# XinMing0411/AC-VAE

Hardware: AMD Instinct MI355X
Metric: train-step captions/s (and audio-sec/s) at B=32, 1/2/4/8 MI355X (higher is better)
Workload: dtype f32

## Files before the change

### acvae_amd/_lib.py

```python
import ctypes
import os
import re
import threading

import numpy as np
import torch

from . import streams

_HERE = os.path.dirname(os.path.abspath(__file__))
HEADER = os.path.join(os.path.dirname(_HERE), "include", "acvae_hip.h")
LIB_PATH = os.path.join(_HERE, "libacvae_hip.so")

_CT = {"int": ctypes.c_int, "int64_t": ctypes.c_int64, "float": ctypes.c_float, "double": ctypes.c_double,
       "uint64_t": ctypes.c_uint64}
ERRORS = {-1: "ACVAE_EINVAL (bad dims / null pointer)", -2: "ACVAE_EALIGN (alignment)",
          -3: "ACVAE_EUNSUPPORTED", -4: "ACVAE_EWORKSPACE (workspace too small)"}


def parse_header(path=HEADER):
    src = open(path).read()
    src = re.sub(r"/\*.*?\*/", "", src, flags=re.S)
    protos = {}
    for m in re.finditer(r"\b(int|int64_t)\s+(acvae_\w+)\s*\(([^)]*)\)\s*;", src):
# ... 5 lines not shown
                if "*" in a:
                    alist.append((a.split("*")[-1].strip(), ctypes.c_void_p))
                else:
                    toks = a.replace("const ", "").split()
                    alist.append((toks[-1], _CT[toks[0]]))
        protos[name] = (_CT[ret], alist)
    enums = {}
    for m in re.finditer(r"enum\s+\w*\s*\{([^}]*)\}", src):
        val = -1
        for item in m.group(1).split(","):
            item = item.strip()
            if not item:
                continue
            if "=" in item:
                k, v = item.split("=")
                val = int(v.strip(), 0)
                enums[k.strip()] = val
            else:
                val += 1
                enums[item] = val
    return protos, enums


PROTOS, ENUMS = parse_header()
_defs = dict(re.findall(r"#define\s+(ACVAE_\w+)\s+(\d+)", open(HEADER).read()))
ENUMS_TEXT_N = int(_defs["ACVAE_TEXT_NPARAMS"])
ENC_NPARAMS = int(_defs["ACVAE_ENC_NPARAMS"])
ENC_BF16 = int(_defs["ACVAE_ENC_BF16"])
FLAG_NO_PERSIST = int(_defs["ACVAE_FLAG_NO_PERSIST"])
FLAG_DEFER_PARAM_GRADS = int(_defs["ACVAE_FLAG_DEFER_PARAM_GRADS"])
FLAG_NO_ATTN_SPLIT = int(_defs["ACVAE_FLAG_NO_ATTN_SPLIT"])
FLAG_TEST_STALL = int(_defs["ACVAE_FLAG_TEST_STALL"])
FLAG_ROLLOUT_GRAD = int(_defs["ACVAE_FLAG_ROLLOUT_GRAD"])
_lib = None


class options:
    persist = os.environ.get("ACVAE_DECODE_PERSIST", "1") != "0"
    defer = os.environ.get("ACVAE_DECODE_DEFER", "1") != "0"
    attn_split = True
    test_stall = False


class override:
    _lock = threading.Lock()
    _open = []
    _base = None

    def __init__(self, **kw):
        self.kw = kw

    @staticmethod
    def _apply():
        vals = dict(override._base)
        for o in override._open:
            vals.update(o.kw)
        for k, v in vals.items():
            setattr(options, k, v)

    def __enter__(self):
        with override._lock:
            if not override._open:
                override._base = {k: v for k, v in vars(options).items() if not k.startswith("_")}
            override._open.append(self)
            override._apply()
        return self

    def __exit__(self, *exc):
        with override._lock:
            override._open.remove(self)
            override._apply()
        return False


def call_flags(defer=False):
    f = 0
    if not options.persist:
        f |= FLAG_NO_PERSIST
    if not options.attn_split:
        f |= FLAG_NO_ATTN_SPLIT
    if options.test_stall:
        f |= FLAG_TEST_STALL
    if defer and options.defer:
        f |= FLAG_DEFER_PARAM_GRADS
    return f


def use_library(path):
    global LIB_PATH
    if _lib is not None:
        raise RuntimeError("acvae_amd._lib.use_library() must come before the first library call")
    LIB_PATH = os.path.abspath(path)


def lib():
    global _lib
    if _lib is None:
        if not os.path.exists(LIB_PATH):
            raise RuntimeError(f"{LIB_PATH} not built: run `python -c 'import __graft_entry__ as g; g.build()'` "
                               "(the AC-VAE HIP path has no CPU fallback)")
        _lib = ctypes.CDLL(LIB_PATH)
        for name, (ret, args) in PROTOS.items():
            fn = getattr(_lib, name)
            fn.restype = ret
            fn.argtypes = [t for _, t in args]
    return _lib


def ptr_table(tensors):
    return (ctypes.c_void_p * len(tensors))(*[None if t is None else t.data_ptr() for t in tensors])


def _conv(x):
    if isinstance(x, torch.Tensor):
        return x.data_ptr()
# ... 199 lines not shown
```

### acvae_amd/csrc/conv.h

```cpp
#pragma once
#include <hip/hip_runtime.h>
#include <stdint.h>
#include "common.h"
#include "job_table.h"
#include "bn_bwd.h"

struct DropoutSpec {
  float p;
  const uint8_t* mask;
  uint64_t seed;
  uint32_t site;
};

enum { UP_PLAIN = 0, UP_POOL = 1, UP_DROP = 2 };

namespace acvae {
int conv3x3_igemm(const float* X, const float* scale, const float* shift, const float* Wp, float* Y, float* partials,
                  int N, int H, int W, int Cin, int Cout, hipStream_t st);
int conv_partials_rows(int N, int H, int W);
int conv3x3_igemm_bf16(const bf16_t* X, const float* scale, const float* shift, const bf16_t* Wp, bf16_t* Y,
                       float* partials, int N, int H, int W, int Cin, int Cout, hipStream_t st);
long conv3x3_wgrad_bf16_slab_floats(int N, int H, int W, int Cin, int Cout);
int conv3x3_wgrad_bf16_splits(int N, int H, int W, int Cin, int Cout);
int conv3x3_wgrad_bf16_launch(const bf16_t* dY, const bf16_t* X, const float* scale, const float* shift, float* slab, int N,
// ... 51 lines not shown
bool colsum_batch_plan(ColsumBatch& b, long dpart_doubles, long* dsum_doubles);
int conv1_first_blocks(int N, int T);
template <class TY>
int conv1_first_fwd(const float* x, const float* scale0, const float* shift0, const float* W1, TY* Y,
                    float* partials, int N, int T, int F, hipStream_t st);
template <class TY>
int conv1_first_bwd(const float* x, const float* scale0, const float* shift0, const float* mean0, const float* invstd0,
                    const float* W1, const TY* dY, float* dw_part, float* bn_part, float* dW1, float* dgamma0,
                    float* dbeta0, double* dpart, int N, int T, int F, hipStream_t st, const BnBwdApply* bn = nullptr);
template <class T>
int bn_relu_pool(const T* Y, const float* scale, const float* shift, T* P, int N, int H, int W, int C,
                 DropoutSpec drop, hipStream_t st, bool pool = true);
int bn_bwd_blocks(int N, int H, int W, int C);
template <class T>
int bn_bwd(const T* Y, const T* dO, int upstream, const float* scale, const float* shift, const float* mean,
           const float* invstd, float* partials, float* sum_g, float* sum_gy, T* dY, double* dpart, int N, int H,
           int W, int C, DropoutSpec drop, hipStream_t st, bool batch_stats = true, int ready_rows = 0);
template <class T>
int bn_bwd_sums(const T* Y, const T* dO, int upstream, const float* scale, const float* shift, const float* mean,
                const float* invstd, float* partials, float* sum_g, float* sum_gy, double* dpart, int N, int H, int W, int C,
                DropoutSpec drop, hipStream_t st, int ready_rows = 0);
template <class T>
int relu_mask(const T* Y, const float* scale, const float* shift, uint8_t* out, int N, int H, int W, int C, hipStream_t st);
template <class T>
int freq_mean(const T* P, float* out, long rows, int Fp, int C, hipStream_t st);
template <class T>
int freq_mean_bwd(const float* dae, T* dP, long rows, int Fp, int C, hipStream_t st);
int time_pool(const float* ae, float* out, int N, int S, int C, DropoutSpec drop, hipStream_t st);
int relu_dropout(float* x, int total, DropoutSpec drop, hipStream_t st);
}

int acvae_gemm_nt_dual(const float* A1, int64_t lda1, const float* B1, int64_t ldb1, int K1, const float* A2,
                       int64_t lda2, const float* B2, int64_t ldb2, int K2, const float* bias, float* C, int64_t ldc,
                       int M, int N, int accumulate, hipStream_t st, float* skws = nullptr);
int acvae_gemm_nt_pair(const float* A0, int64_t lda0, const float* B0, int64_t ldb0, int K0, const float* bias0, float* C0,
                       int64_t ldc0, int N0, int acc0, const float* A1, int64_t lda1, const float* B1, int64_t ldb1, int K1,
                       const float* bias1, float* C1, int64_t ldc1, int N1, int acc1, int M, hipStream_t st);
constexpr int TN_TICKETS = 256;
int acvae_gemm_tn_fused(const float* A, int64_t lda, const float* B, int64_t ldb, float* C, int64_t ldc, int M, int N, int K,
                        int accumulate, float* ws, int64_t ws_bytes, hipStream_t st);
struct TnJob {
  const float* A; long lda; const float* B; long ldb; float* C; long ldc;
  int M, N, K, k_per, slices, gx, gy, tk0;
  long slab0;
};
using TnGroup = acvae::RangeTable<TnJob, 8, int>;
bool acvae_gemm_tn_group_add(TnGroup& g, const float* A, long lda, const float* B, long ldb, float* C, long ldc, int M, int N,
                             int K);
long acvae_gemm_tn_group_plan(TnGroup& g);
int acvae_gemm_tn_group(TnGroup& g, float* ws, int64_t ws_bytes, hipStream_t st);
long acvae_skinny_ws_floats();
long acvae_skinny_ticket_words();
int acvae_skinny_ws_reset(float* ws, hipStream_t st);
struct TransposeJob { const float* in; long ld_in; float* out; long ld_out; int rows, cols; };
using TransposeBatch = acvae::RangeTable<TransposeJob, 12, int>;
int acvae_transpose_batch(TransposeBatch& b, hipStream_t st);
```

### acvae_amd/csrc/decoder.hip

```cpp
#include <cstdlib>
#include <vector>
#include "common.h"
#include "constrain.h"
#include "conv.h"
#include "rnn.h"
#include "decode_persist.h"
#include "text_common.h"

namespace {

inline int gemm2(const float* A1, long lda1, const float* B1, long ldb1, int K1, const float* A2, long lda2,
                 const float* B2, long ldb2, int K2, const float* bias, float* C, long ldc, int M, int N, int acc,
                 const Ctx& st) {
  if (M <= 64)
    return acvae_gemm_nt_dual(A1, lda1, B1, ldb1, K1, A2, lda2, B2, ldb2, K2, bias, C, ldc, M, N, acc, st.s, st.skws);
  ACVAE_TRY(acvae_gemm_nt_dual(A1, lda1, B1, ldb1, K1, nullptr, 0, nullptr, 0, 0, bias, C, ldc, M, N, acc, st.s, st.skws));
  return acvae_gemm_nt_dual(A2, lda2, B2, ldb2, K2, nullptr, 0, nullptr, 0, 0, nullptr, C, ldc, M, N, 1, st.s, st.skws);
}
struct TnWs { float* p; long bytes; };
inline int gemm_tn(const float* A, long lda, const float* B, long ldb, float* C, long ldc, int M, int N, int K, TnWs ws,
                   hipStream_t st) {
  return acvae_gemm_tn_fused(A, lda, B, ldb, C, ldc, M, N, K, 0, ws.p, ws.bytes, st);
}
struct TnBatch {
// ... 526 lines not shown
  if (truncate && (sample_method == ACVAE_SAMPLE_GREEDY || (flags & ACVAE_FLAG_ROLLOUT_GRAD))) return ACVAE_EINVAL;
  if (emb_keep && !(emb_drop_p > 0.f && emb_drop_p <= 1.f)) return ACVAE_EINVAL;
  if (sample_method != ACVAE_SAMPLE_GREEDY &&
      ((sample_method != ACVAE_SAMPLE_GUMBEL && sample_method != ACVAE_SAMPLE_MULTINOMIAL) || !sample_noise ||
       !(temp > 0.f)))
    return ACVAE_EINVAL;
  DecLayout L;
  ACVAE_TRY(dec_layout(N, Tc, S, E, H, A, V, Eenc, L));
  if (!params || !mem_in || !mem_lens || !eps_p || !logits || !outputs || !seqs || !sampled_logprobs || !attn_w ||
      !p_means || !p_logs || !p_z || !saved_v || !scratch_v)
    return ACVAE_EINVAL;
  const bool train = caps != nullptr;
  const bool rollout_grad = !train && (flags & ACVAE_FLAG_ROLLOUT_GRAD);
  if (train && (!lens1 || !q_z || !ss_flags_host || !dis_flags_host || !p_means_utt)) return ACVAE_EINVAL;
  if (train && H != E) return ACVAE_EUNSUPPORTED;
  if (saved_bytes < L.saved_total * 4 || scratch_bytes < dec_scratch_floats(L) * 4) return ACVAE_EWORKSPACE;
  float* sv = (float*)saved_v;
  float* sc = (float*)scratch_v;
  auto P = [&](int i) { return (const float*)params[i]; };
  const int R = N * Tc, Hp = E;
  const bool has_ln = Eenc != E || params[TP_LN_W] != nullptr;
  bool teacher = train, prior_feeds_decoder = !train;
  if (train)
    for (int t = 0; t < Tc; ++t) {
      teacher = teacher && ss_flags_host[t] != 0;
      prior_feeds_decoder = prior_feeds_decoder || dis_flags_host[t] != 0;
    }
  Ctx st{(hipStream_t)stream, sc + L.skws};
  const Fork fork{st.s, (aux_stream && teacher) ? (hipStream_t)aux_stream : st.s};
  Ctx sp{fork.aux, sc + L.skws_p};
  acvae::PdPlan pd_plan{};
  const bool persist_fwd = teacher && !prior_feeds_decoder && !(flags & ACVAE_FLAG_NO_PERSIST) && H == E &&
                           acvae::decode_fwd_resident(N, Tc, S, E, H, A, pd_plan);
  const bool attws_ready = !persist_fwd && L.attfws_bytes > 0;
  {
    acvae::ZeroBatch zb;
    zb_skinny(zb, st.skws); zb_skinny(zb, sp.skws);
    if (attws_ready) { zb.add(sc + L.attfws_d, 256); zb.add(sc + L.attfws_p, 256); }
    if (persist_fwd) { zb.add(sc + L.pd_cnt, pd_plan.counter_words); flags |= ACVAE_FLAG_INT_CNT_ZEROED; }
    zb.add(sc + L.h0, (long)N * (H > Hp ? H : Hp));
    ACVAE_TRY(acvae::zero_batch(zb, st.s));
  }

  int64_t* words = (int64_t*)(sv + L.words);
  const float* mem = has_ln ? sv + L.mem : mem_in;
  float* encproj_d = sv + L.encproj_d;
  float* encproj_p = sv + L.encproj_p;
  float* qd = sv + L.qd;
  float* qp = sv + L.qp;
  float* attw_p = sv + L.attw_p;
  float* rnn_d = sv + L.rnn_d;
  float* rnn_p = sv + L.rnn_p;
  float* gi_d = sc + L.gi_d;
  float* gh_d = sc + L.gh_d;
  float* gates_p = sc + L.gates_p;
  float* ml = sc + L.ml;
  float* zeros = sc + L.h0;
  uint8_t* unfinished = (uint8_t*)(sv + L.unfinished);
  const long ld3E = (long)Tc * 3 * E;

  if (has_ln) ACVAE_TRY(gemm(mem_in, Eenc, P(TP_LN_W), Eenc, P(TP_LN_B), sv + L.mem, E, N * S, E, Eenc, 0, st));
  auto encproj_prior = [&](const Ctx& c) -> int {
    return gemm(mem, E, P(TP_P_ATT_W) + E, 2 * E, P(TP_P_ATT_B), encproj_p, E, N * S, E, E, 0, c);
  };
  auto encproj_dec = [&]() -> int {
    return gemm(mem, E, P(TP_DEC_ATT_W) + H, E + H, P(TP_DEC_ATT_B), encproj_d, A, N * S, A, E, 0, st);
  };

  auto rows_of = [&](int cnt) { return cnt == Tc ? R : N; };
  auto ldof = [&](int cnt, long C) { return cnt == Tc ? C : (long)Tc * C; };
  auto prior_pre = [&](int t0, int cnt) -> int {
    const int M = rows_of(cnt);
    ACVAE_TRY(acvae::embed_gather(words + t0, cnt == Tc ? 1 : Tc, P(TP_P_EMB), V, rnn_p + (long)t0 * 3 * E,
                                  ldof(cnt, 3 * E), M, E, sp));
    ACVAE_TRY(gemm(rnn_p + (long)t0 * 3 * E, ldof(cnt, 3 * E), P(TP_P_ATT_W), 2 * E, nullptr, qp + (long)t0 * E,
                   ldof(cnt, E), M, E, E, 0, sp));
    ACVAE_TRY(acvae_attn_fwd(qp + (long)t0 * E, (long)Tc * E, E, encproj_p, mem, mem_lens, P(TP_P_ATT_V),
                             rnn_p + (long)t0 * 3 * E + E, ld3E, 3 * E, attw_p + (long)t0 * S, (long)Tc * S, S, N, cnt, S,
                             E, E, (cnt == 1 && attws_ready) ? sc + L.attfws_p : nullptr, L.attfws_bytes, sp, flags));
    ACVAE_TRY(gemm(rnn_p + (long)t0 * 3 * E, ldof(cnt, 3 * E), P(TP_P_WIH), 3 * E, P(TP_P_BIH),
                   gates_p + (long)t0 * 4 * Hp, ldof(cnt, 4 * Hp), M, 4 * Hp, 2 * E, 0, sp));
    return ACVAE_OK;
  };
  float* hp_all = sv + L.hp_all;
  float* c_all = sv + L.c_all;
  float* hpprev = sv + L.hpprev;
  float* lstm_save = sv + L.lstm_save;
  auto prior_step = [&](int t) -> int {
    const float* hprev = t ? hp_all + (long)(t - 1) * Hp : zeros;
    const long ldh = t ? (long)Tc * Hp : Hp;
    const float* cprev = t ? c_all + (long)(t - 1) * Hp : nullptr;
    if (t == 0) ACVAE_TRY(acvae::copy_rows(rnn_p + 2 * E, ld3E, nullptr, 0, N, E, sp));
    ACVAE_TRY(gemm2(rnn_p + (long)t * 3 * E + 2 * E, ld3E, P(TP_P_WIH) + 2 * E, 3 * E, E, hprev, ldh, P(TP_P_WHH), Hp,
                    Hp, P(TP_P_BHH), gates_p + (long)t * 4 * Hp, (long)Tc * 4 * Hp, N, 4 * Hp, 1, sp));
    ACVAE_TRY(acvae::lstm_fwd(gates_p + (long)t * 4 * Hp, (long)Tc * 4 * Hp, cprev, (long)Tc * Hp,
                              hp_all + (long)t * Hp, (long)Tc * Hp, c_all + (long)t * Hp, (long)Tc * Hp,
                              lstm_save + (long)t * 5 * Hp, (long)Tc * 5 * Hp, N, Hp, sp));
    ACVAE_TRY(gemm(hp_all + (long)t * Hp, (long)Tc * Hp, P(TP_P_ML_W), Hp, P(TP_P_ML_B), ml, 2 * E, N, 2 * E, Hp, 0, sp));
    float* z2 = (t + 1 < Tc) ? rnn_p + (long)(t + 1) * 3 * E + 2 * E : nullptr;
    ACVAE_TRY(acvae_reparam_fwd(ml, 2 * E, eps_p + (long)t * N * E, E, p_means + (long)t * E, p_logs + (long)t * E,
                                p_z + (long)t * E, (long)Tc * E, z2, ld3E, N, E, sp));
    return ACVAE_OK;
  };
  auto dec_pre = [&](int t0, int cnt) -> int {
    const int M = rows_of(cnt);
    ACVAE_TRY(acvae::embed_gather(words + t0, cnt == Tc ? 1 : Tc, P(TP_DEC_EMB), V, rnn_d + (long)t0 * 3 * E,
                                  ldof(cnt, 3 * E), M, E, st));
    if (emb_keep)
      ACVAE_TRY(acvae::dropout_rows(rnn_d + (long)t0 * 3 * E, ld3E, 3 * E, emb_keep + (long)t0 * N * E, E, (long)N * E,
                                    emb_drop_p < 1.f ? 1.f / (1.f - emb_drop_p) : 0.f, N, cnt, E, st));
    if (cnt == Tc && train && !prior_feeds_decoder) {
      ACVAE_TRY(acvae::copy_rows(rnn_d + 2 * E, 3 * E, q_z, E, R, E, st));
    } else {
      for (int t = t0; t < t0 + cnt; ++t) {
        const float* zsrc = (train && !dis_flags_host[t]) ? q_z : p_z;
        ACVAE_TRY(acvae::copy_rows(rnn_d + (long)t * 3 * E + 2 * E, ld3E, zsrc + (long)t * E, (long)Tc * E, N, E, st));
      }
    }
    ACVAE_TRY(gemm2(rnn_d + (long)t0 * 3 * E, ldof(cnt, 3 * E), P(TP_DEC_WIH), 3 * E, E,
                    rnn_d + (long)t0 * 3 * E + 2 * E, ldof(cnt, 3 * E), P(TP_DEC_WIH) + 2 * E, 3 * E, E, P(TP_DEC_BIH),
                    gi_d + (long)t0 * 3 * H, ldof(cnt, 3 * H), M, 3 * H, 0, st));
    return ACVAE_OK;
  };
  float* gru_save = sv + L.gru_save;
  float* hprev_d = sv + L.hprev_d;
  const bool pair_ok = N <= 64;
  auto dec_step = [&](int t) -> int {
    const float* hprev = t ? outputs + (long)(t - 1) * H : zeros;
    const long ldh = t ? (long)Tc * H : H;
    if (pair_ok) {
      ACVAE_TRY(acvae_gemm_nt_pair(hprev, ldh, P(TP_DEC_ATT_W), E + H, H, nullptr, qd + (long)t * A, (long)Tc * A, A, 0,
                                   hprev, ldh, P(TP_DEC_WHH), H, H, P(TP_DEC_BHH), gh_d, 3 * H, 3 * H, 0, N, st));
    } else {
      ACVAE_TRY(gemm(hprev, ldh, P(TP_DEC_ATT_W), E + H, nullptr, qd + (long)t * A, (long)Tc * A, N, A, H, 0, st));
      ACVAE_TRY(gemm(hprev, ldh, P(TP_DEC_WHH), H, P(TP_DEC_BHH), gh_d, 3 * H, N, 3 * H, H, 0, st));
    }
    ACVAE_TRY(acvae_attn_fwd(qd + (long)t * A, (long)Tc * A, A, encproj_d, mem, mem_lens, P(TP_DEC_ATT_V),
// ... 11 lines not shown
    TransposeBatch tb;
    tb.add({P(TP_DEC_CLS_W), H, sv + L.wt_cls, V, V, H});
    tb.add({P(TP_DEC_WIH), 3 * E, sv + L.wt_dih, 3 * H, 3 * H, 3 * E});
    tb.add({P(TP_DEC_WHH), H, sv + L.wt_dhh, 3 * H, 3 * H, H});
    tb.add({P(TP_DEC_ATT_W), E + H, sv + L.wt_datt, A, A, E + H});
    tb.add({P(TP_P_WIH), 3 * E, sv + L.wt_pih, 4 * Hp, 4 * Hp, 3 * E});
    tb.add({P(TP_P_WHH), Hp, sv + L.wt_phh, 4 * Hp, 4 * Hp, Hp});
    tb.add({P(TP_P_ML_W), Hp, sv + L.wt_pml, 2 * E, 2 * E, Hp});
    tb.add({P(TP_P_ATT_W), 2 * E, sv + L.wt_patt, E, E, 2 * E});
    if (train) tb.add({P(TP_MLO_W), H, sv + L.wt_mlo, 2 * E, 2 * E, H});
    return acvae_transpose_batch(tb, ts);
  };
  float* lse = sv + L.lse;
  auto classify = [&](int t0, int cnt) -> int {
    const int M = rows_of(cnt);
    ACVAE_TRY(gemm(outputs + (long)t0 * H, ldof(cnt, H), P(TP_DEC_CLS_W), H, P(TP_DEC_CLS_B), logits + (long)t0 * V,
                   ldof(cnt, V), M, V, H, 0, st));
    if (con.on())
      ACVAE_TRY(acvae::constrain_rows(logits + (long)t0 * V, (long)Tc * V, seqs, Tc, t0, N, V, end_idx, con, st.s));
    ACVAE_TRY(acvae_row_logsoftmax_argmax(logits + (long)t0 * V, (long)Tc * V, V, seqs + t0, sampled_logprobs + t0,
                                          lse + t0, Tc, 1, N, cnt, V, st));
    if (truncate)
      ACVAE_TRY(acvae_sample_next_word_truncated(logits + (long)t0 * V, (long)Tc * V, V, sample_noise + (long)t0 * N * V,
                                                 V, (long)N * V, sample_method, temp, seqs + t0, sampled_logprobs + t0,
                                                 Tc, 1, N, cnt, V, top_k, top_p, kept ? kept + t0 : nullptr, st));
    else if (sample_method != ACVAE_SAMPLE_GREEDY)
      ACVAE_TRY(acvae_sample_next_word(logits + (long)t0 * V, (long)Tc * V, V, sample_noise + (long)t0 * N * V, V,
                                       (long)N * V, sample_method, temp, seqs + t0, sampled_logprobs + t0, Tc, 1, N, cnt,
                                       V, st));
    return ACVAE_OK;
  };

  if (teacher) {
    ACVAE_TRY(acvae::gather_words(caps, ld_caps, 1, words, N, Tc, st));
    ACVAE_TRY(fork.begin());
    ACVAE_TRY(encproj_prior(sp));
    ACVAE_TRY(encproj_dec());
    ACVAE_TRY(prior_pre(0, Tc));
    if (prior_feeds_decoder) {
      for (int t = 0; t < Tc; ++t) ACVAE_TRY(prior_step(t));
      ACVAE_TRY(fork.join());
      ACVAE_TRY(dec_pre(0, Tc));
      for (int t = 0; t < Tc; ++t) ACVAE_TRY(dec_step(t));
    } else if (persist_fwd) {
      ACVAE_TRY(dec_pre(0, Tc));
      ACVAE_TRY(acvae::copy_rows(rnn_p + 2 * E, ld3E, nullptr, 0, N, E, sp));
      ACVAE_TRY(fork.join());
      PdParams pd{};
      pd.w_att = P(TP_DEC_ATT_W); pd.w_hh = P(TP_DEC_WHH); pd.b_hh = P(TP_DEC_BHH); pd.w_ih = P(TP_DEC_WIH);
      pd.att_v = P(TP_DEC_ATT_V);
      pd.pw_ih = P(TP_P_WIH); pd.pw_hh = P(TP_P_WHH); pd.pb_hh = P(TP_P_BHH); pd.w_ml = P(TP_P_ML_W); pd.b_ml = P(TP_P_ML_B);
      pd.encproj = encproj_d; pd.mem = mem; pd.mem_lens = mem_lens; pd.gi = gi_d; pd.gates_p = gates_p;
      pd.eps_p = eps_p; pd.zeros = zeros;
      pd.qd = qd; pd.gh = gh_d; pd.rnn_d = rnn_d; pd.attn_w = attn_w; pd.outputs = outputs; pd.gru_save = sv + L.gru_save;
      pd.hprev_d = sv + L.hprev_d; pd.rnn_p = rnn_p; pd.hp_all = sv + L.hp_all; pd.c_all = sv + L.c_all;
      pd.lstm_save = sv + L.lstm_save; pd.p_means = p_means; pd.p_logs = p_logs; pd.p_z = p_z;
      pd.cnt = (unsigned*)(sc + L.pd_cnt);
      ACVAE_TRY(acvae::decode_persist_fwd(pd, pd_plan, st.s, flags));
    } else {
      ACVAE_TRY(dec_pre(0, Tc));
      for (int t = 0; t < Tc; ++t) {
        ACVAE_TRY(prior_step(t));
        ACVAE_TRY(dec_step(t));
      }
    }
    ACVAE_TRY(transposes(sp.s));
    ACVAE_TRY(classify(0, Tc));
// ... 57 lines not shown
                                          void* stream, void* aux_stream, int sample_method, float temp,
                                          const float* sample_noise, const uint8_t* emb_keep, float emb_drop_p, int flags,
                                          int top_k, float top_p, int32_t* kept) {
  return decode_fwd_driver(params, mem_in, mem_lens, caps, ld_caps, lens1, q_z, eps_p, ss_flags_host, dis_flags_host, logits,
                           outputs, seqs, sampled_logprobs, attn_w, p_means, p_logs, p_z, p_means_utt, h_final, hp_final,
                           cp_final, saved_v, saved_bytes, scratch_v, scratch_bytes, N, Tc, S, E, H, A, V, Eenc, start_idx,
                           end_idx, stream, aux_stream, sample_method, temp, sample_noise, emb_keep, emb_drop_p, flags,
                           top_k, top_p, kept, acvae::Constraints{});
}

extern "C" int acvae_decode_fwd_constrained(const void* const* params, const float* mem_in, const int64_t* mem_lens,
                                            const int64_t* caps, int64_t ld_caps, const int64_t* lens1, const float* q_z,
                                            const float* eps_p, const int* ss_flags_host, const int* dis_flags_host,
                                            float* logits, float* outputs, int64_t* seqs, float* sampled_logprobs,
                                            float* attn_w, float* p_means, float* p_logs, float* p_z, float* p_means_utt,
                                            float* h_final, float* hp_final, float* cp_final, void* saved_v,
                                            int64_t saved_bytes, void* scratch_v, int64_t scratch_bytes, int N, int Tc,
                                            int S, int E, int H, int A, int V, int Eenc, int start_idx, int end_idx,
                                            void* stream, void* aux_stream, int sample_method, float temp,
                                            const float* sample_noise, const uint8_t* emb_keep, float emb_drop_p, int flags,
                                            int top_k, float top_p, int32_t* kept, float repetition_penalty,
                                            int no_repeat_ngram_size, int min_length, const int* suppress_host,
                                            int n_suppress) {
  acvae::Constraints con;
  con.repetition_penalty = repetition_penalty; con.no_repeat_ngram_size = no_repeat_ngram_size;
  con.min_length = min_length; con.suppress = suppress_host; con.n_suppress = n_suppress;
  return decode_fwd_driver(params, mem_in, mem_lens, caps, ld_caps, lens1, q_z, eps_p, ss_flags_host, dis_flags_host, logits,
                           outputs, seqs, sampled_logprobs, attn_w, p_means, p_logs, p_z, p_means_utt, h_final, hp_final,
                           cp_final, saved_v, saved_bytes, scratch_v, scratch_bytes, N, Tc, S, E, H, A, V, Eenc, start_idx,
                           end_idx, stream, aux_stream, sample_method, temp, sample_noise, emb_keep, emb_drop_p, flags,
                           top_k, top_p, kept, con);
}

extern "C" int acvae_decode_bwd_defers(const int* dis_flags_host, int Tc, void* stream, void* aux_stream, int flags) {
  if (!(flags & ACVAE_FLAG_DEFER_PARAM_GRADS) || !aux_stream || aux_stream == stream || !dis_flags_host) return 0;
  for (int t = 0; t < Tc; ++t)
    if (dis_flags_host[t] != 0) return 0;
  return 1;
}

extern "C" int acvae_decode_bwd(const void* const* params, void* const* grads, const float* mem_in,
                                const int64_t* mem_lens, const int64_t* lens1, const float* eps_p,
                                const int* dis_flags_host, const float* outputs, const float* attn_w,
                                const float* p_logs, const float* d_logits, const float* d_outputs_ext,
                                const float* d_p_means, const float* d_p_logs, const float* d_p_z,
                                const float* d_p_means_utt, float* d_mem_in, float* d_q_z, void* saved_v,
                                int64_t saved_bytes, void* scratch_v, int64_t scratch_bytes, int N, int Tc, int S, int E,
                                int H, int A, int V, int Eenc, void* stream, void* aux_stream, const uint8_t* emb_keep,
                                float emb_drop_p, int flags) {
  if (emb_keep && !(emb_drop_p > 0.f && emb_drop_p <= 1.f)) return ACVAE_EINVAL;
  DecLayout L;
  ACVAE_TRY(dec_layout(N, Tc, S, E, H, A, V, Eenc, L));
  const bool rollout = (flags & ACVAE_FLAG_ROLLOUT_GRAD) != 0;
  if (!params || !grads || !mem_in || !mem_lens || !eps_p || !outputs || !attn_w || !p_logs || !d_mem_in || !saved_v ||
      !scratch_v)
    return ACVAE_EINVAL;
  if (rollout ? d_p_means_utt != nullptr : (!lens1 || !dis_flags_host || !d_q_z)) return ACVAE_EINVAL;
  if (saved_bytes < L.saved_total * 4 || scratch_bytes < dec_scratch_floats(L) * 4) return ACVAE_EWORKSPACE;
  float* sv = (float*)saved_v;
  float* sc = (float*)scratch_v;
  std::vector<int> rollout_flags;
  if (rollout) {
    rollout_flags.assign(Tc, 1);
    dis_flags_host = rollout_flags.data();
  }
  bool prior_feeds_decoder = false;
  for (int t = 0; t < Tc; ++t) prior_feeds_decoder = prior_feeds_decoder || dis_flags_host[t] != 0;
  Ctx st{(hipStream_t)stream, sc + L.skws};
  const Fork fork{st.s, aux_stream ? (hipStream_t)aux_stream : st.s};
  Ctx sp{fork.aux, sc + L.skws_p};
  auto P = [&](int i) { return (const float*)params[i]; };
  auto G = [&](int i) { return (float*)grads[i]; };
  const int R = N * Tc, Hp = E;
  const bool defer = acvae_decode_bwd_defers(dis_flags_host, Tc, stream, aux_stream, flags) != 0;
  const bool has_ln = Eenc != E || params[TP_LN_W] != nullptr;
  TnWs tn{sc + L.tn, L.tn_floats * 4};
  TnWs tn_p{sc + L.tn_p, L.tn_p_floats * 4};
  double* dpart = (double*)(sc + L.dpart);
  double* dpart_p = (double*)(sc + L.dpart_p);
  const acvae::PbPlan pb_plan = acvae::decode_bwd_plan(N, Tc, S, E, H, A);
  const bool persist_bwd = !prior_feeds_decoder && !(flags & ACVAE_FLAG_NO_PERSIST) && acvae::decode_bwd_resident(pb_plan);
  {
    acvae::ZeroBatch zb;
    zb_skinny(zb, st.skws); zb_skinny(zb, sp.skws); zb_colsum(zb, dpart); zb_colsum(zb, dpart_p); zb_tn(zb, tn); zb_tn(zb, tn_p);
    if (persist_bwd) {
      zb.add(sc + L.pd_cnt_b, pb_plan.counter_words);
      zb.add(sc + L.dmem_p, (long)N * S * E);
      if (pb_plan.rc_splits > 1) zb.add(sc + L.dqd, (long)R * A);
      flags |= ACVAE_FLAG_INT_CNT_ZEROED;
    }
    zb.add(G(TP_DEC_EMB), (long)V * E); zb.add(G(TP_P_EMB), (long)V * E);
    ACVAE_TRY(acvae::zero_batch(zb, st.s));
  }
  const int64_t* words = (const int64_t*)(sv + L.words);
  const float* mem = has_ln ? sv + L.mem : mem_in;
  float* rnn_d = sv + L.rnn_d;
  float* rnn_p = sv + L.rnn_p;

  float *wt_cls = sv + L.wt_cls, *wt_dih = sv + L.wt_dih, *wt_dhh = sv + L.wt_dhh, *wt_datt = sv + L.wt_datt;
  float *wt_pih = sv + L.wt_pih, *wt_phh = sv + L.wt_phh, *wt_pml = sv + L.wt_pml, *wt_patt = sv + L.wt_patt;
  float *wt_mlo = sv + L.wt_mlo, *wt_ln = sc + L.wt_ln;
  int64_t* words_c = (int64_t*)(sc + L.words_c);
  ACVAE_TRY(acvae::gather_words(words, Tc, 1, words_c, N, Tc, st));
  ACVAE_TRY(fork.begin());

  float* d_out = sc + L.d_out;
  if (d_outputs_ext) ACVAE_TRY(acvae::copy_rows(d_out, H, d_outputs_ext, H, R, H, st));
  else ACVAE_TRY(zero(d_out, (long)R * H, st));
// ... 37 lines not shown
  float* dh = sc + L.dh_a;
  float* dh2 = sc + L.dh_b;
  const float* gru_save = sv + L.gru_save;
  const float* hprev_d = sv + L.hprev_d;
  const float* qd = sv + L.qd;
  auto dec_begin = [&]() -> int {
    ACVAE_TRY(zero(dencproj, (long)N * S * A, st));
    ACVAE_TRY(zero(dvpart, (long)N * A, st));
    ACVAE_TRY(zero(dmem, (long)N * S * E, st));
    ACVAE_TRY(zero(dh, (long)N * H, st));
    return ACVAE_OK;
  };
  float* drnn = sc + L.drnn;
  float* dz_dec = sc + L.dz_dec;
  int dv_rows = N;
  auto dec_bptt = [&](int t) -> int {
    ACVAE_TRY(acvae::gru_bwd(dh, H, d_out + (long)t * H, (long)Tc * H, gru_save + (long)t * 4 * H, (long)Tc * 4 * H,
                             hprev_d + (long)t * H, (long)Tc * H, dgi + (long)t * 3 * H, (long)Tc * 3 * H,
                             dgh + (long)t * 3 * H, (long)Tc * 3 * H, dh2, H, nullptr, t, N, H, st));
    ACVAE_TRY(gemm(dgi + (long)t * 3 * H, (long)Tc * 3 * H, wt_dih + (long)E * 3 * H, 3 * H, nullptr, dctx, E, N, E,
                   3 * H, 0, st));
    ACVAE_TRY(acvae_attn_bwd(dctx, E, 0, qd + (long)t * A, (long)Tc * A, A, sv + L.encproj_d, mem, mem_lens,
                             P(TP_DEC_ATT_V), attn_w + (long)t * S, (long)Tc * S, S, dqd + (long)t * A, (long)Tc * A, A,
                             dencproj, dmem, dvpart, sc + L.attws, L.attws_bytes, N, 1, S, A, E, st));
    ACVAE_TRY(gemm2(dgh + (long)t * 3 * H, (long)Tc * 3 * H, wt_dhh, 3 * H, 3 * H, dqd + (long)t * A, (long)Tc * A,
                    wt_datt, A, A, nullptr, dh2, H, N, H, 1, st));
    float* tmp = dh; dh = dh2; dh2 = tmp;
    return ACVAE_OK;
  };
  auto dec_memgrad = [&]() -> int {
    return gemm(dencproj, A, wt_datt + (long)H * A, A, nullptr, dmem, E, N * S, E, A, 1, st);
  };
  auto dec_dz = [&](const Ctx& c) -> int {
    ACVAE_TRY(gemm(dgi, 3 * H, wt_dih + (long)2 * E * 3 * H, 3 * H, nullptr, dz_dec, E, R, E, 3 * H, 0, c));
    if (!d_q_z) return ACVAE_OK;
    if (!prior_feeds_decoder) {
      ACVAE_TRY(acvae::copy_rows(d_q_z, E, dz_dec, E, R, E, c));
    } else {
      for (int t = 0; t < Tc; ++t)
        ACVAE_TRY(acvae::copy_rows(d_q_z + (long)t * E, (long)Tc * E, dis_flags_host[t] ? nullptr : dz_dec + (long)t * E,
                                   (long)Tc * E, N, E, c));
    }
    return ACVAE_OK;
  };
  auto dec_tn = [&](TnBatch& tb) -> int {
    ACVAE_TRY(tb.add(dgi, 3 * H, rnn_d, 3 * E, G(TP_DEC_WIH), 3 * E, 3 * H, 3 * E, R));
    ACVAE_TRY(tb.add(dgh, 3 * H, hprev_d, H, G(TP_DEC_WHH), H, 3 * H, H, R));
    ACVAE_TRY(tb.add(dqd, A, hprev_d, H, G(TP_DEC_ATT_W), E + H, A, H, R));
    return tb.add(dencproj, A, mem, E, G(TP_DEC_ATT_W) + H, E + H, A, E, N * S);
  };
  auto dec_params = [&](const Ctx& c, TnWs ws, double* dp, bool with_dz = true, bool with_tn = true) -> int {
    if (with_tn) {
      TnBatch tb{{}, ws, c};
      ACVAE_TRY(dec_tn(tb));
      ACVAE_TRY(tb.launch());
    }
    {
      acvae::ColsumBatch cb;
      cb.add({dgi, R, 3 * H, G(TP_DEC_BIH)}); cb.add({dgh, R, 3 * H, G(TP_DEC_BHH)});
      cb.add({dencproj, N * S, A, G(TP_DEC_ATT_B)}); cb.add({dvpart, dv_rows, A, G(TP_DEC_ATT_V)});
      ACVAE_TRY(acvae::colsum_batch(cb, dp, L.dpart_doubles, c));
    }
    ACVAE_TRY(gemm(dgi, 3 * H, wt_dih, 3 * H, nullptr, drnn, E, R, E, 3 * H, 0, c));
    if (emb_keep)
      ACVAE_TRY(acvae::dropout_rows(drnn, (long)Tc * E, E, emb_keep, E, (long)N * E, emb_drop_p < 1.f ? 1.f / (1.f - emb_drop_p) : 0.f, N, Tc, E, c));
    if (with_dz) ACVAE_TRY(dec_dz(c));
// ... 21 lines not shown
  auto prior_begin = [&]() -> int {
  for (int t = 0; t < Tc; ++t) {
    ACVAE_TRY(acvae::copy_rows(dpz + (long)t * E, (long)Tc * E, d_p_z ? d_p_z + (long)t * E : nullptr, (long)Tc * E, N, E,
                               sp));
    if (dis_flags_host[t])
      ACVAE_TRY(acvae::add_rows(dpz + (long)t * E, (long)Tc * E, dz_dec + (long)t * E, (long)Tc * E, N, E, sp));
  }
  ACVAE_TRY(zero(dmem_p, (long)N * S * E, sp));
  ACVAE_TRY(zero(dhp, (long)N * Hp, sp));
  ACVAE_TRY(zero(dc, (long)N * Hp, sp));
  ACVAE_TRY(zero(dlz, (long)N * E, sp));
    return ACVAE_OK;
  };
  auto prior_bptt = [&](int t) -> int {
    ACVAE_TRY(acvae::add_rows(dlz, E, dpz + (long)t * E, (long)Tc * E, N, E, sp));
    ACVAE_TRY(acvae_reparam_bwd(dlz, E, d_p_means ? d_p_means + (long)t * E : nullptr,
                                d_p_logs ? d_p_logs + (long)t * E : nullptr, (long)Tc * E, p_logs + (long)t * E,
                                (long)Tc * E, eps_p + (long)t * N * E, E, dml_all + (long)t * 2 * E, (long)Tc * 2 * E, N,
                                E, sp));
    ACVAE_TRY(gemm(dml_all + (long)t * 2 * E, (long)Tc * 2 * E, wt_pml, 2 * E, nullptr, dhp, Hp, N, Hp, 2 * E, 1, sp));
    ACVAE_TRY(acvae::lstm_bwd(dhp, Hp, dc, Hp, lstm_save + (long)t * 5 * Hp, (long)Tc * 5 * Hp,
                              t ? c_all + (long)(t - 1) * Hp : nullptr, (long)Tc * Hp, dgates + (long)t * 4 * Hp,
                              (long)Tc * 4 * Hp, dc2, Hp, N, Hp, sp));
    ACVAE_TRY(gemm(dgates + (long)t * 4 * Hp, (long)Tc * 4 * Hp, wt_phh, 4 * Hp, nullptr, dhp2, Hp, N, Hp, 4 * Hp, 0, sp));
    ACVAE_TRY(gemm(dgates + (long)t * 4 * Hp, (long)Tc * 4 * Hp, wt_pih + (long)2 * E * 4 * Hp, 4 * Hp, nullptr, dlz2, E,
                   N, E, 4 * Hp, 0, sp));
    float* tmp = dhp; dhp = dhp2; dhp2 = tmp;
    tmp = dc; dc = dc2; dc2 = tmp;
    tmp = dlz; dlz = dlz2; dlz2 = tmp;
    return ACVAE_OK;
  };
  float* dqp = sc + L.dqp;
  auto prior_memgrad = [&]() -> int {
    ACVAE_TRY(gemm(dgates, 4 * Hp, wt_pih, 4 * Hp, nullptr, drnn_p, 3 * E, R, 2 * E, 4 * Hp, 0, sp));
    ACVAE_TRY(zero(dencproj_p, (long)N * S * E, sp));
    ACVAE_TRY(zero(dvpart_p, (long)N * E, sp));
    ACVAE_TRY(acvae_attn_bwd(drnn_p + E, (long)Tc * 3 * E, 3 * E, sv + L.qp, (long)Tc * E, E, sv + L.encproj_p, mem,
                             mem_lens, P(TP_P_ATT_V), sv + L.attw_p, (long)Tc * S, S, dqp, (long)Tc * E, E, dencproj_p,
                             dmem_p, dvpart_p, sc + L.attws_p, L.attws_bytes, N, Tc, S, E, E, sp));
    return gemm(dencproj_p, E, wt_patt + (long)E * E, E, nullptr, dmem_p, E, N * S, E, E, 1, sp);
  };
  auto prior_tn_bptt = [&](TnBatch& tb) -> int {
    ACVAE_TRY(tb.add(dgates, 4 * Hp, rnn_p, 3 * E, G(TP_P_WIH), 3 * E, 4 * Hp, 3 * E, R));
    ACVAE_TRY(tb.add(dgates, 4 * Hp, hpprev, Hp, G(TP_P_WHH), Hp, 4 * Hp, Hp, R));
    return tb.add(dml_all, 2 * E, hp_all, Hp, G(TP_P_ML_W), Hp, 2 * E, Hp, R);
  };
  auto prior_params = [&](bool with_bptt_tn = true) -> int {
    {
      TnBatch tb{{}, tn_p, sp};
      if (with_bptt_tn) ACVAE_TRY(prior_tn_bptt(tb));
      ACVAE_TRY(tb.add(dqp, E, rnn_p, 3 * E, G(TP_P_ATT_W), 2 * E, E, E, R));
      ACVAE_TRY(tb.add(dencproj_p, E, mem, E, G(TP_P_ATT_W) + E, 2 * E, E, E, N * S));
      ACVAE_TRY(tb.launch());
    }
    {
      acvae::ColsumBatch cb;
      cb.add({dml_all, R, 2 * E, G(TP_P_ML_B)}); cb.add({dgates, R, 4 * Hp, G(TP_P_BIH), G(TP_P_BHH)});
      cb.add({dencproj_p, N * S, E, G(TP_P_ATT_B)}); cb.add({dvpart_p, N, E, G(TP_P_ATT_V)});
      ACVAE_TRY(acvae::colsum_batch(cb, dpart_p, L.dpart_doubles, sp));
    }
    ACVAE_TRY(gemm(dqp, E, wt_patt, E, nullptr, drnn_p, 3 * E, R, E, E, 1, sp));
    return acvae::embed_scatter(words_c, drnn_p, 3 * E, G(TP_P_EMB), V, R, E, sp);
  };
  bool early_tn = false;
  if (prior_feeds_decoder) {
    ACVAE_TRY(dec_begin());
    for (int t = Tc - 1; t >= 0; --t) ACVAE_TRY(dec_bptt(t));
    ACVAE_TRY(dec_memgrad());
    ACVAE_TRY(dec_params(st, tn, dpart));
    if (fork.on()) ACVAE_TRY(Fork::edge(st.s, sp.s));
    ACVAE_TRY(prior_begin());
    for (int t = Tc - 1; t >= 0; --t) ACVAE_TRY(prior_bptt(t));
    ACVAE_TRY(prior_memgrad());
    ACVAE_TRY(prior_params());
  } else if (persist_bwd) {
    PbParams pb{};
    pb.wt_dhh = wt_dhh; pb.wt_datt = wt_datt; pb.wt_dih = wt_dih; pb.wt_phh = wt_phh; pb.wt_pih = wt_pih; pb.wt_pml = wt_pml;
    pb.att_v = P(TP_DEC_ATT_V);
    pb.encproj = sv + L.encproj_d; pb.mem = mem; pb.qd = qd; pb.attn_w = attn_w; pb.gru_save = gru_save; pb.hprev_d = hprev_d;
    pb.lstm_save = lstm_save; pb.c_all = c_all; pb.p_logs = p_logs; pb.eps_p = eps_p; pb.mem_lens = mem_lens;
    pb.d_out = d_out; pb.d_p_z = d_p_z; pb.d_p_means = d_p_means; pb.d_p_logs = d_p_logs;
    pb.dgi = dgi; pb.dgh = dgh; pb.dqd = dqd; pb.dctx = drnn;
    pb.dencproj = dencproj; pb.dmem = dmem; pb.dvpart = dvpart; pb.dgates = dgates; pb.dml_all = dml_all; pb.dhp = dhp;
    float* part = sc + L.pd_part;
    pb.dctx_part = part + pb_plan.dctx_part_off; pb.dhp_part = part + pb_plan.dhp_part_off; pb.dml_part = part + pb_plan.dml_part_off;
    pb.cnt = (unsigned*)(sc + L.pd_cnt_b);
    pb.dqd_part = sc + L.pd_dqd; pb.ctx = rnn_d + E;
    ACVAE_TRY(acvae::decode_persist_bwd(pb, pb_plan, st.s, flags));
    dv_rows = pb_plan.dv_rows;
    ACVAE_TRY(dec_memgrad());
    if (fork.on()) ACVAE_TRY(Fork::edge(st.s, sp.s));
    ACVAE_TRY(prior_memgrad());
    if (!defer) {
      ACVAE_TRY(dec_params(st, tn, dpart));
      ACVAE_TRY(prior_params());
    } else {
      TnBatch tb{{}, tn, st.s};
      ACVAE_TRY(dec_tn(tb));
      ACVAE_TRY(prior_tn_bptt(tb));
      ACVAE_TRY(tb.launch());
      early_tn = true;
    }
  } else {
    ACVAE_TRY(dec_begin());
    ACVAE_TRY(prior_begin());
    for (int t = Tc - 1; t >= 0; --t) {
      ACVAE_TRY(dec_bptt(t));
      ACVAE_TRY(prior_bptt(t));
    }
    ACVAE_TRY(dec_memgrad());
    ACVAE_TRY(prior_memgrad());
    if (!defer) {
      ACVAE_TRY(dec_params(st, tn, dpart));
      ACVAE_TRY(prior_params());
    }
  }
  ACVAE_TRY(fork.join());
  ACVAE_TRY(acvae::add_rows(dmem, E, dmem_p, E, N * S, E, st));
  if (has_ln) {
    ACVAE_TRY(transp(P(TP_LN_W), Eenc, wt_ln, E, E, Eenc, st));
    ACVAE_TRY(gemm(dmem, E, wt_ln, E, nullptr, d_mem_in, Eenc, N * S, Eenc, E, 0, st));
    ACVAE_TRY(gemm_tn(dmem, E, mem_in, Eenc, G(TP_LN_W), Eenc, E, Eenc, N * S, tn, st));
    ACVAE_TRY(acvae::colsum2(dmem, N * S, E, dpart, G(TP_LN_B), nullptr, 0, st));
  } else {
    ACVAE_TRY(acvae::copy_rows(d_mem_in, E, dmem, E, N * S, E, st));
  }
  if (defer) {
    ACVAE_TRY(dec_dz(st));
    ACVAE_TRY(Fork::edge(st.s, sp.s));
    ACVAE_TRY(dec_params(sp, tn_p, dpart_p, false, !early_tn));
    ACVAE_TRY(prior_params(!early_tn));
  }
  return ACVAE_OK;
}

extern "C" int acvae_caps_to_long(const float* caps, int64_t* out, int64_t n, void* stream) {
  if (!caps || !out || n <= 0) return ACVAE_EINVAL;
  return acvae::caps_to_long(caps, out, (long)n, (hipStream_t)stream);
}
```

### acvae_amd/csrc/gemm.hip

```cpp
#include <cstdint>
#include <cstdlib>
#include "mfma_tile.h"
#include "../../include/acvae_hip.h"
#include "conv.h"

namespace {
using namespace mfma;

template <int BN, bool VEC4>
__global__ __launch_bounds__(nt_threads<128>(), 2) void gemm_nt_kernel(const float* __restrict__ A, long lda,
                                                                     const float* __restrict__ B, long ldb,
                                                                     const float* __restrict__ bias,
                                                                     float* __restrict__ C, long ldc, int M, int N,
                                                                     int K, int accumulate) {
  __shared__ NtSmem<128, BN> sm;
  PlainLoader<VEC4, 4> al{A, lda, M, K};
  PlainLoader<VEC4, BN / 32> bl{B, ldb, N, K};
  PlainEpilogue ep{C, ldc, bias, accumulate};
  int bm, bn;
  xcd_tile(gridDim.x, gridDim.y, bm, bn);
  nt_block<128, BN>(al, bl, M, N, K, bm, bn, ep, sm);
}

template <int WM, int WN, bool VEC4>
// ... 275 lines not shown
int acvae_gemm_nt_pair(const float* A0, int64_t lda0, const float* B0, int64_t ldb0, int K0, const float* bias0, float* C0,
                       int64_t ldc0, int N0, int acc0, const float* A1, int64_t lda1, const float* B1, int64_t ldb1, int K1,
                       const float* bias1, float* C1, int64_t ldc1, int N1, int acc1, int M, hipStream_t st) {
  if (!A0 || !B0 || !C0 || !A1 || !B1 || !C1 || M <= 0 || M > 64 || N0 <= 0 || N1 <= 0 || K0 <= 0 || K1 <= 0)
    return ACVAE_EINVAL;
  const bool vec = vec_ok(A0, lda0, K0) && vec_ok(B0, ldb0, K0) && vec_ok(A1, lda1, K1) && vec_ok(B1, ldb1, K1);
  const SkProblem p0{A0, lda0, B0, ldb0, K0, bias0, C0, ldc0, N0, acc0}, p1{A1, lda1, B1, ldb1, K1, bias1, C1, ldc1, N1, acc1};
  const int nx0 = cdiv(N0, 32);
  dim3 grid(nx0 + cdiv(N1, 32), cdiv(M, 32));
  if (vec) hipLaunchKernelGGL(gemm_skinny_pair_kernel<true>, grid, dim3(SK_THREADS), 0, st, p0, p1, nx0, M);
  else hipLaunchKernelGGL(gemm_skinny_pair_kernel<false>, grid, dim3(SK_THREADS), 0, st, p0, p1, nx0, M);
  ACVAE_LAUNCH_CHECK();
  return ACVAE_OK;
}

static int skinny_plan(int M, int N, int Ktot, bool dual, bool have_ws) {
  const long big_blocks = (long)cdiv(M, 128) * cdiv(N, N <= 64 ? 64 : 128);
  if (!(M <= 64 || dual || (big_blocks < 100 && M <= 4096))) return 0;
  const int tiles = cdiv(N, 32) * cdiv(M, 32);
  int S = 1;
  if (have_ws && tiles <= 16 && Ktot >= 1024) {
    S = 128 / tiles;
    const int maxs = Ktot / 256;
    if (S > maxs) S = maxs;
    if (S > 8) S = 8;
    if (S < 1) S = 1;
    if ((long)tiles * S > SK_MAX_TILES) S = 1;
  }
  return S;
}

int acvae_gemm_nt_dual(const float* A1, int64_t lda1, const float* B1, int64_t ldb1, int K1, const float* A2,
                       int64_t lda2, const float* B2, int64_t ldb2, int K2, const float* bias, float* C, int64_t ldc,
                       int M, int N, int accumulate, hipStream_t st, float* skws) {
  if (!A1 || !B1 || !C || M <= 0 || N <= 0 || K1 <= 0) return ACVAE_EINVAL;
  if (A2 && (!B2 || K2 <= 0)) return ACVAE_EINVAL;
  bool vec = vec_ok(A1, lda1, K1) && vec_ok(B1, ldb1, K1);
  if (A2) vec = vec && vec_ok(A2, lda2, K2) && vec_ok(B2, ldb2, K2);
  const int S = skinny_plan(M, N, K1 + (A2 ? K2 : 0), A2 != nullptr, skws != nullptr);
  if (S > 0) {
    dim3 grid(cdiv(N, 32), cdiv(M, 32), S);
    unsigned* cnt = (unsigned*)skws;
    float* slabs = skws ? skws + SK_MAX_TILES : nullptr;
    if (vec)
      hipLaunchKernelGGL(gemm_skinny_kernel<true>, grid, dim3(SK_THREADS), 0, st, A1, lda1, B1, ldb1, K1, A2, lda2, B2,
                         ldb2, K2, bias, C, ldc, M, N, accumulate, slabs, cnt);
    else
      hipLaunchKernelGGL(gemm_skinny_kernel<false>, grid, dim3(SK_THREADS), 0, st, A1, lda1, B1, ldb1, K1, A2, lda2,
                         B2, ldb2, K2, bias, C, ldc, M, N, accumulate, slabs, cnt);
    ACVAE_LAUNCH_CHECK();
    return ACVAE_OK;
  }
  const bool bn64 = (N <= 64);
  dim3 grid(cdiv(M, 128), cdiv(N, bn64 ? 64 : 128));
#define LAUNCH_NT(BN_, V_)                                                                                     \
  hipLaunchKernelGGL((gemm_nt_kernel<BN_, V_>), grid, dim3(nt_threads<128>()), 0, st, A1, lda1, B1, ldb1, bias, C, ldc, M, \
                     N, K1, accumulate)
  if (bn64) { if (vec) LAUNCH_NT(64, true); else LAUNCH_NT(64, false); }
  else      { if (vec) LAUNCH_NT(128, true); else LAUNCH_NT(128, false); }
#undef LAUNCH_NT
  ACVAE_LAUNCH_CHECK();
  return ACVAE_OK;
}

extern "C" int acvae_gemm_nt(const float* A, int64_t lda, const float* B, int64_t ldb, const float* bias, float* C,
                             int64_t ldc, int M, int N, int K, int accumulate, void* stream) {
  return acvae_gemm_nt_dual(A, lda, B, ldb, K, nullptr, 0, nullptr, 0, 0, bias, C, ldc, M, N, accumulate,
                            (hipStream_t)stream, nullptr);
}

static int tn_splits(int M, int N, int K) {
  const long tiles = (long)cdiv(M, 128) * cdiv(N, 128);
  int s = (int)(256 / (tiles > 0 ? tiles : 1));
  const int maxs = cdiv(K, 4 * BKT);
  if (s > maxs) s = maxs;
  if (s < 1) s = 1;
  if (s > 256) s = 256;
  return s;
}

extern "C" int64_t acvae_gemm_tn_workspace_bytes(int M, int N, int K) {
  const int s = tn_splits(M, N, K);
  return s > 1 ? (int64_t)s * M * N * (int64_t)sizeof(float) : 0;
}

extern "C" int acvae_gemm_tn(const float* A, int64_t lda, const float* B, int64_t ldb, float* C, int64_t ldc, int M,
// ... 97 lines not shown
  if (g.n <= 0) return ACVAE_OK;
  const long slab = acvae_gemm_tn_group_plan(g);
  if (slab < 0 || (slab > 0 && (!ws || ws_bytes < ((int64_t)TN_TICKETS + slab) * (int64_t)sizeof(float)))) return ACVAE_EWORKSPACE;
  hipLaunchKernelGGL(gemm_tn_group_kernel, dim3(g.start[g.n]), dim3(256), 0, st, g, ws + TN_TICKETS,
                     reinterpret_cast<unsigned*>(ws));
  ACVAE_LAUNCH_CHECK();
  return ACVAE_OK;
}

extern "C" int acvae_transpose(const float* in, int64_t ld_in, float* out, int64_t ld_out, int rows, int cols,
                               void* stream) {
  if (!in || !out || rows <= 0 || cols <= 0) return ACVAE_EINVAL;
  hipLaunchKernelGGL(transpose_kernel, dim3(cdiv(cols, 32), cdiv(rows, 32)), dim3(32, 8), 0, (hipStream_t)stream, in,
                     ld_in, out, ld_out, rows, cols);
  ACVAE_LAUNCH_CHECK();
  return ACVAE_OK;
}

extern "C" int64_t acvae_gemm_nt_splitk_workspace_bytes(void) { return acvae_skinny_ws_floats() * (int64_t)sizeof(float); }
extern "C" int acvae_gemm_nt_split_plan(int M, int N, int K1, int K2, int with_ws) {
  if (M <= 0 || N <= 0 || K1 <= 0 || K2 < 0) return ACVAE_EINVAL;
  return skinny_plan(M, N, K1 + K2, K2 > 0, with_ws != 0);
}
extern "C" int acvae_gemm_nt_dual_ws(const float* A1, int64_t lda1, const float* B1, int64_t ldb1, int K1, const float* A2,
                                     int64_t lda2, const float* B2, int64_t ldb2, int K2, const float* bias, float* C,
                                     int64_t ldc, int M, int N, int accumulate, float* ws, int64_t ws_bytes, int reset_tickets,
                                     void* stream) {
  if (!A1 || !B1 || !C || M <= 0 || N <= 0 || K1 <= 0 || (A2 && (!B2 || K2 <= 0))) return ACVAE_EINVAL;
  if (ws && ws_bytes < acvae_gemm_nt_splitk_workspace_bytes()) return ACVAE_EWORKSPACE;
  hipStream_t st = (hipStream_t)stream;
  if (ws && reset_tickets) ACVAE_TRY(acvae_skinny_ws_reset(ws, st));
  return acvae_gemm_nt_dual(A1, lda1, B1, ldb1, K1, A2, lda2, B2, ldb2, K2, bias, C, ldc, M, N, accumulate, st, ws);
}
extern "C" int acvae_gemm_nt_pair_c(const float* A0, int64_t lda0, const float* B0, int64_t ldb0, int K0, const float* bias0,
                                    float* C0, int64_t ldc0, int N0, int acc0, const float* A1, int64_t lda1, const float* B1,
                                    int64_t ldb1, int K1, const float* bias1, float* C1, int64_t ldc1, int N1, int acc1, int M,
                                    void* stream) {
  return acvae_gemm_nt_pair(A0, lda0, B0, ldb0, K0, bias0, C0, ldc0, N0, acc0, A1, lda1, B1, ldb1, K1, bias1, C1, ldc1, N1,
                            acc1, M, (hipStream_t)stream);
}
extern "C" int64_t acvae_gemm_tn_fused_workspace_bytes(int M, int N, int K) {
  if (M <= 0 || N <= 0 || K <= 0) return -1;
  const int s = tn_splits(M, N, K);
  return s > 1 ? (int64_t)TN_TICKETS * 4 + (int64_t)s * M * N * (int64_t)sizeof(float) : 0;
}
extern "C" int acvae_gemm_tn_fused_plan(int M, int N, int K, int64_t ws_bytes) {
  if (M <= 0 || N <= 0 || K <= 0) return ACVAE_EINVAL;
  return tn_fused_slices(M, N, K, ws_bytes > 0, ws_bytes, nullptr);
}
extern "C" int acvae_gemm_tn_fused_c(const float* A, int64_t lda, const float* B, int64_t ldb, float* C, int64_t ldc, int M,
                                     int N, int K, int accumulate, float* ws, int64_t ws_bytes, int reset_tickets,
                                     void* stream) {
  if (!A || !B || !C || M <= 0 || N <= 0 || K <= 0) return ACVAE_EINVAL;
  hipStream_t st = (hipStream_t)stream;
  if (ws && reset_tickets && ws_bytes >= (int64_t)TN_TICKETS * 4)
    if (hipMemsetAsync(ws, 0, TN_TICKETS * sizeof(unsigned), st) != hipSuccess) return (int)hipGetLastError();
  return acvae_gemm_tn_fused(A, lda, B, ldb, C, ldc, M, N, K, accumulate, ws, ws_bytes, st);
}

static int tn_group_shapes(int n, const int* M, const int* N, const int* K, TnGroup& g) {
  if (n <= 0 || n > TnGroup::capacity || !M || !N || !K) return ACVAE_EINVAL;
  const float* none = reinterpret_cast<const float*>(16);
  for (int l = 0; l < n; ++l)
    if (!acvae_gemm_tn_group_add(g, none, 4, none, 4, const_cast<float*>(none), 4, M[l], N[l], K[l])) return ACVAE_EINVAL;
  return ACVAE_OK;
}
// ... 24 lines not shown
```

### acvae_amd/csrc/losses.hip

```cpp
#include "common.h"
#include "dbs_rules.h"
#include "../../include/acvae_hip.h"

namespace {

constexpr int EW_THREADS = 256;
constexpr int RED_BLOCKS_MAX = 1024;

__global__ void reparam_fwd_kernel(const float* __restrict__ ml, long ld_ml, const float* __restrict__ eps,
                                   long ld_eps, float* __restrict__ mean, float* __restrict__ logv,
                                   float* __restrict__ z, long ld_out, float* __restrict__ z2, long ld_z2, int rows,
                                   int E) {
  const long total = (long)rows * E;
  for (long i = blockIdx.x * (long)blockDim.x + threadIdx.x; i < total; i += (long)gridDim.x * blockDim.x) {
    const int r = (int)(i / E), e = (int)(i % E);
    const float mu = ml[r * ld_ml + e], lv = ml[r * ld_ml + E + e];
    const float zz = eps[r * ld_eps + e] * expf(.5f * lv) + mu;
    mean[r * ld_out + e] = mu;
    logv[r * ld_out + e] = lv;
    z[r * ld_out + e] = zz;
    if (z2) z2[r * ld_z2 + e] = zz;
  }
}

__global__ void reparam_bwd_kernel(const float* __restrict__ dz, long ld_dz, const float* __restrict__ dmean_ext,
                                   const float* __restrict__ dlog_ext, long ld_ext, const float* __restrict__ logv,
                                   long ld_lv, const float* __restrict__ eps, long ld_eps, float* __restrict__ dml,
                                   long ld_dml, int rows, int E) {
  const long total = (long)rows * E;
  for (long i = blockIdx.x * (long)blockDim.x + threadIdx.x; i < total; i += (long)gridDim.x * blockDim.x) {
    const int r = (int)(i / E), e = (int)(i % E);
    const float g = dz ? dz[r * ld_dz + e] : 0.f;
    float dm = g, dl = g * eps[r * ld_eps + e] * .5f * expf(.5f * logv[r * ld_lv + e]);
    if (dmean_ext) dm += dmean_ext[r * ld_ext + e];
    if (dlog_ext) dl += dlog_ext[r * ld_ext + e];
    dml[r * ld_dml + e] = dm;
    dml[r * ld_dml + E + e] = dl;
  }
}

__global__ void final_sum_kernel(const float* __restrict__ partials, int n, float scale, float* __restrict__ out) {
  __shared__ float red[16];
  double acc = 0.0;
  for (int i = threadIdx.x; i < n; i += blockDim.x) acc += (double)partials[i];
  acc = wave_sum_d(acc);
  __shared__ double redd[16];
  if ((threadIdx.x & 63) == 0) redd[threadIdx.x >> 6] = acc;
  __syncthreads();
  if (threadIdx.x == 0) {
    double t = 0.0;
    for (int i = 0; i < (int)(blockDim.x >> 6); ++i) t += redd[i];
    out[0] = (float)(t * (double)scale);
  }
  (void)red;
}

__device__ __forceinline__ float kl_elem(float mu1, float lv1, float mu2, float lv2) {
  const float d = mu1 - mu2;
  return lv2 * .5f - lv1 * .5f + (expf(lv1) + d * d) / (2.f * expf(lv2)) - .5f;
}

__global__ __launch_bounds__(EW_THREADS) void kl_fwd_kernel(const float* __restrict__ mu1,
                                                            const float* __restrict__ lv1,
                                                            const float* __restrict__ mu2,
                                                            const float* __restrict__ lv2, float* __restrict__ partials,
                                                            long n) {
  __shared__ float red[16];
  float acc = 0.f;
  const long n4 = n >> 2;
  for (long i = blockIdx.x * (long)EW_THREADS + threadIdx.x; i < n4; i += (long)gridDim.x * EW_THREADS) {
    const float4 a = reinterpret_cast<const float4*>(mu1)[i], b = reinterpret_cast<const float4*>(lv1)[i];
    const float4 c = reinterpret_cast<const float4*>(mu2)[i], d = reinterpret_cast<const float4*>(lv2)[i];
    acc += kl_elem(a.x, b.x, c.x, d.x) + kl_elem(a.y, b.y, c.y, d.y) + kl_elem(a.z, b.z, c.z, d.z) +
           kl_elem(a.w, b.w, c.w, d.w);
  }
  if (blockIdx.x == 0)
    for (long i = (n4 << 2) + threadIdx.x; i < n; i += EW_THREADS) acc += kl_elem(mu1[i], lv1[i], mu2[i], lv2[i]);
  acc = block_sum(acc, red);
  if (threadIdx.x == 0) partials[blockIdx.x] = acc;
}

__global__ void kl_bwd_kernel(const float* __restrict__ mu1, const float* __restrict__ lv1,
                              const float* __restrict__ mu2, const float* __restrict__ lv2,
                              const float* __restrict__ grad_out, float inv_rows, float* __restrict__ dmu1,
                              float* __restrict__ dlv1, float* __restrict__ dmu2, float* __restrict__ dlv2, long n) {
  const float g = grad_out[0] * inv_rows;
  for (long i = blockIdx.x * (long)blockDim.x + threadIdx.x; i < n; i += (long)gridDim.x * blockDim.x) {
    const float d = mu1[i] - mu2[i];
    const float v1 = expf(lv1[i]), iv2 = 1.f / expf(lv2[i]);
    if (dmu1) dmu1[i] = g * d * iv2;
    if (dmu2) dmu2[i] = -g * d * iv2;
    if (dlv1) dlv1[i] = g * (-.5f + .5f * v1 * iv2);
    if (dlv2) dlv2[i] = g * (.5f - .5f * (v1 + d * d) * iv2);
  }
}

__global__ __launch_bounds__(EW_THREADS) void mse_fwd_kernel(const float* __restrict__ a, const float* __restrict__ b,
                                                             float* __restrict__ partials, long n) {
  __shared__ float red[16];
  float acc = 0.f;
  for (long i = blockIdx.x * (long)EW_THREADS + threadIdx.x; i < n; i += (long)gridDim.x * EW_THREADS) {
    const float d = a[i] - b[i];
    acc += d * d;
  }
  acc = block_sum(acc, red);
  if (threadIdx.x == 0) partials[blockIdx.x] = acc;
}
__global__ void mse_bwd_kernel(const float* __restrict__ a, const float* __restrict__ b,
                               const float* __restrict__ grad_out, float scale, float* __restrict__ da,
                               float* __restrict__ db, long n) {
  const float g = grad_out[0] * scale;
  for (long i = blockIdx.x * (long)blockDim.x + threadIdx.x; i < n; i += (long)gridDim.x * blockDim.x) {
    const float d = g * (a[i] - b[i]);
    if (da) da[i] = d;
    if (db) db[i] = -d;
  }
}

__global__ __launch_bounds__(EW_THREADS) void row_stats_kernel(const float* __restrict__ logits, long ld_n, long ld_t,
                                                               int64_t* __restrict__ argmax,
                                                               float* __restrict__ max_logprob,
                                                               float* __restrict__ lse, long o_sn, long o_st, int T,
                                                               int V) {
  __shared__ float red[16];
  __shared__ int redi[16];
  const int n = blockIdx.x / T, t = blockIdx.x % T;
  const float* x = logits + n * ld_n + t * ld_t;
  float m = -INFINITY;
  int mi = 0x7fffffff;
  for (int c = threadIdx.x; c < V; c += EW_THREADS) {
    const float v = x[c];
    if (v > m) { m = v; mi = c; }
  }
#pragma unroll
  for (int o = 32; o > 0; o >>= 1) {
    const float om = __shfl_xor(m, o, 64);
    const int oi = __shfl_xor(mi, o, 64);
    if (om > m || (om == m && oi < mi)) { m = om; mi = oi; }
  }
  const int w = threadIdx.x >> 6;
  if ((threadIdx.x & 63) == 0) { red[w] = m; redi[w] = mi; }
  __syncthreads();
  m = red[0]; mi = redi[0];
  for (int i = 1; i < EW_THREADS / 64; ++i)
    if (red[i] > m || (red[i] == m && redi[i] < mi)) { m = red[i]; mi = redi[i]; }
  float s = 0.f;
  for (int c = threadIdx.x; c < V; c += EW_THREADS) s += expf(x[c] - m);
  s = block_sum(s, red);
  if (threadIdx.x == 0) {
// ... 180 lines not shown
    if (in && (v > best || bi == 0x7fffffff)) { best = v; bi = c; }
  };
  if constexpr (REG) {
#pragma unroll
    for (int i = 0; i < VPT; ++i)
      if (tid + i * EW_THREADS < V) take(key[i], tid + i * EW_THREADS, sc[i]);
  } else {
    for (int c = tid; c < V; c += EW_THREADS) take(trunc_key(x[c]), c, score(x[c], z[c]));
  }
#pragma unroll
  for (int o = 32; o > 0; o >>= 1) {
    const float ob = __shfl_xor(best, o, 64);
    const int oi = __shfl_xor(bi, o, 64);
    if (ob > best || (ob == best && oi < bi)) { best = ob; bi = oi; }
  }
  __syncthreads();
  const int w = tid >> 6;
  if ((tid & 63) == 0) { red[w] = best; redi[w] = bi; pi[0][w] = nk; }
  __syncthreads();
  if (tid == 0) {
    best = red[0]; bi = redi[0]; nk = pi[0][0];
    for (int i = 1; i < EW_THREADS / 64; ++i) {
      if (red[i] > best || (red[i] == best && redi[i] < bi)) { best = red[i]; bi = redi[i]; }
      nk += pi[0][i];
    }
    if (bi < 0 || bi >= V) bi = 0;
    const long o = n * o_sn + t * o_st;
    w_out[o] = bi;
    if (lp_out) lp_out[o] = (x[bi] - m) - ls;
    if (kept_out) kept_out[o] = nk;
  }
}

__global__ __launch_bounds__(EW_THREADS) void ce_rows_kernel(const float* __restrict__ logits, long ld_n, long ld_t,
                                                             const int64_t* __restrict__ targets, long tg_sn,
                                                             const int64_t* __restrict__ lens1,
                                                             const float* __restrict__ lse, float smoothing,
                                                             float* __restrict__ loss_rows, int T, int V) {
  __shared__ float red[16];
  const int n = blockIdx.x / T, t = blockIdx.x % T;
  const long o = (long)n * T + t;
  if (lens1 && t >= (int)lens1[n]) {
    if (threadIdx.x == 0) loss_rows[o] = 0.f;
    return;
  }
  const float* x = logits + n * ld_n + t * ld_t;
  const float l = lse[o];
  float sumlp = 0.f;
  if (smoothing != 0.f) {
    for (int c = threadIdx.x; c < V; c += EW_THREADS) sumlp += x[c] - l;
    sumlp = block_sum(sumlp, red);
  }
  if (threadIdx.x == 0) {
    const float lpt = x[targets[n * tg_sn + t]] - l;
    loss_rows[o] = -((1.f - smoothing) * lpt + (smoothing != 0.f ? smoothing / (float)(V - 1) * (sumlp - lpt) : 0.f));
  }
}

__global__ void ce_reduce_kernel(const float* __restrict__ loss_rows, const int64_t* __restrict__ lens1, int N, int T,
                                 int mean, float* __restrict__ out) {
  __shared__ double redd[16];
  double acc = 0.0;
  for (int i = threadIdx.x; i < N * T; i += blockDim.x) acc += (double)loss_rows[i];
  acc = wave_sum_d(acc);
  if ((threadIdx.x & 63) == 0) redd[threadIdx.x >> 6] = acc;
  __syncthreads();
  if (threadIdx.x == 0) {
    double t = 0.0;
    for (int i = 0; i < (int)(blockDim.x >> 6); ++i) t += redd[i];
    if (mean) {
      long cnt = 0;
      for (int n = 0; n < N; ++n) cnt += lens1 ? (lens1[n] < T ? lens1[n] : T) : T;
      t /= (double)cnt;
    }
    out[0] = (float)t;
  }
}

__global__ __launch_bounds__(EW_THREADS) void ce_bwd_kernel(const float* __restrict__ logits, long ld_n, long ld_t,
                                                            const int64_t* __restrict__ targets, long tg_sn,
                                                            const int64_t* __restrict__ lens1,
                                                            const float* __restrict__ lse, float smoothing,
                                                            int reduction, const float* __restrict__ grad_out,
                                                            const float* __restrict__ grad_rows,
                                                            float* __restrict__ dlogits, int N, int T, int V) {
  const int n = blockIdx.x / T, t = blockIdx.x % T;
  float* d = dlogits + n * ld_n + t * ld_t;
  if (lens1 && t >= (int)lens1[n]) {
    for (int c = threadIdx.x; c < V; c += EW_THREADS) d[c] = 0.f;
    return;
  }
  float g;
  if (reduction == 0) {
    g = grad_rows[(long)n * T + t];
  } else {
    g = grad_out[0];
    if (reduction == 1) {
      long cnt = 0;
      for (int i = 0; i < N; ++i) cnt += lens1 ? (lens1[i] < T ? lens1[i] : T) : T;
      g /= (float)cnt;
    }
  }
  const float* x = logits + n * ld_n + t * ld_t;
  const float l = lse[(long)n * T + t];
  const int tg = (int)targets[n * tg_sn + t];
  const float off = smoothing / (float)(V - 1), on = 1.f - smoothing;
  for (int c = threadIdx.x; c < V; c += EW_THREADS) d[c] = g * (expf(x[c] - l) - (c == tg ? on : off));
}

__global__ __launch_bounds__(EW_THREADS) void scst_loss_kernel(const float* __restrict__ slp,
                                                               const int64_t* __restrict__ seqs,
                                                               const float* __restrict__ reward, int end_idx,
                                                               float* __restrict__ coef, float* __restrict__ loss, int N,
                                                               int T) {
  __shared__ double redd[EW_THREADS / 64];
  const float inv_n = 1.f / (float)N;
  double acc = 0.0;
  for (int i = threadIdx.x; i < N * T; i += EW_THREADS) {
    const int n = i / T, t = i % T;
    const bool live = t == 0 || seqs[i - 1] != (int64_t)end_idx;
    const float c = live ? -reward[n] * inv_n : 0.f;
    coef[i] = c;
    if (c != 0.f) acc += (double)c * (double)slp[i];
  }
  acc = wave_sum_d(acc);
  if ((threadIdx.x & 63) == 0) redd[threadIdx.x >> 6] = acc;
  __syncthreads();
  if (threadIdx.x == 0) {
    double t = 0.0;
    for (int i = 0; i < EW_THREADS / 64; ++i) t += redd[i];
    loss[0] = (float)t;
  }
}

template <bool VEC>
__global__ __launch_bounds__(EW_THREADS) void logprob_bwd_kernel(const float* __restrict__ logits, long ld,
                                                                 const float* __restrict__ lse,
                                                                 const int64_t* __restrict__ seqs,
                                                                 const float* __restrict__ coef,
                                                                 float* __restrict__ dlogits, int V) {
// ... 230 lines not shown
  return ACVAE_OK;
}

__global__ void loss_combine_fwd_kernel(const float* ce, const float* kl, const float* mse, float w_kl, float w_mse, float* out) {
  if (threadIdx.x == 0 && blockIdx.x == 0) {
    float v = ce[0] + w_kl * kl[0];
    if (mse) v = v + w_mse * mse[0];
    out[0] = v;
  }
}
__global__ void loss_combine_bwd_kernel(const float* g, float w_kl, float w_mse, float* g_ce, float* g_kl, float* g_mse) {
  if (threadIdx.x == 0 && blockIdx.x == 0) {
    const float v = g[0];
    g_ce[0] = v;
    g_kl[0] = v * w_kl;
    if (g_mse) g_mse[0] = v * w_mse;
  }
}
extern "C" int acvae_loss_combine_fwd(const float* ce, const float* kl, const float* mse, float w_kl, float w_mse, float* out,
                                      void* stream) {
  if (!ce || !kl || !out) return ACVAE_EINVAL;
  hipLaunchKernelGGL(loss_combine_fwd_kernel, dim3(1), dim3(64), 0, (hipStream_t)stream, ce, kl, mse, w_kl, w_mse, out);
  ACVAE_LAUNCH_CHECK();
  return ACVAE_OK;
}
extern "C" int acvae_loss_combine_bwd(const float* grad_out, float w_kl, float w_mse, float* g_ce, float* g_kl, float* g_mse,
                                      void* stream) {
  if (!grad_out || !g_ce || !g_kl) return ACVAE_EINVAL;
  hipLaunchKernelGGL(loss_combine_bwd_kernel, dim3(1), dim3(64), 0, (hipStream_t)stream, grad_out, w_kl, w_mse, g_ce, g_kl, g_mse);
  ACVAE_LAUNCH_CHECK();
  return ACVAE_OK;
}

extern "C" int acvae_row_logsoftmax_argmax(const float* logits, int64_t ld_n, int64_t ld_t, int64_t* argmax,
                                           float* max_logprob, float* lse, int64_t o_sn, int64_t o_st, int N, int T,
                                           int V, void* stream) {
  if (!logits || N <= 0 || T <= 0 || V <= 0) return ACVAE_EINVAL;
  hipLaunchKernelGGL(row_stats_kernel, dim3(N * T), dim3(EW_THREADS), 0, (hipStream_t)stream, logits, ld_n, ld_t,
                     argmax, max_logprob, lse, o_sn, o_st, T, V);
  ACVAE_LAUNCH_CHECK();
  return ACVAE_OK;
}

__global__ void sample_noise_kernel(float* __restrict__ out, long n, int method, uint64_t seed) {
  for (long i4 = blockIdx.x * (long)blockDim.x + threadIdx.x; i4 * 4 < n; i4 += (long)gridDim.x * blockDim.x) {
    const uint4 r = philox4x32(seed, (uint64_t)i4, 0x5a3d1u);
    const uint32_t w[4] = {r.x, r.y, r.z, r.w};
#pragma unroll
    for (int k = 0; k < 4; ++k) {
      const long i = i4 * 4 + k;
      if (i < n) {
        const float u = (float)(w[k] >> 8) * (1.0f / 16777216.0f);
        out[i] = method == ACVAE_SAMPLE_GUMBEL ? -logf(-logf(u + 1e-20f) + 1e-20f) : fmaxf(-log1pf(-u), 1e-30f);
      }
    }
  }
}

extern "C" int acvae_sample_noise(float* noise, int64_t n, int method, uint64_t seed, void* stream) {
  if (!noise || n <= 0 || (method != ACVAE_SAMPLE_GUMBEL && method != ACVAE_SAMPLE_MULTINOMIAL)) return ACVAE_EINVAL;
  const long blocks = (n / 4 + EW_THREADS - 1) / EW_THREADS;
  hipLaunchKernelGGL(sample_noise_kernel, dim3((unsigned)(blocks > 65536 ? 65536 : (blocks < 1 ? 1 : blocks))), dim3(EW_THREADS), 0,
                     (hipStream_t)stream, noise, (long)n, method, seed);
  ACVAE_LAUNCH_CHECK();
  return ACVAE_OK;
}
// ... 138 lines not shown
```

### acvae_amd/csrc/rnn.h

```cpp
#pragma once
#include <hip/hip_runtime.h>
#include <stdint.h>
#include "job_table.h"
namespace acvae {
int caps_to_long(const float* caps, int64_t* out, long n, hipStream_t st);
int select_word(const int64_t* caps, long ld_caps, const int64_t* seqs, long ld_seqs, int64_t* words, long ld_words,
                int t, int use_caps, int start_idx, int N, hipStream_t st);
int finish_rows(int64_t* seqs, long ld_seqs, uint8_t* unfinished, int t, int end_idx, int N, hipStream_t st);
int embed_gather(const int64_t* words, long w_stride, const float* table, int V, float* out, long ld_out, int rows,
                 int E, hipStream_t st);
int embed_scatter(const int64_t* words_contig, const float* d, long ld_d, float* dtable, int V, int rows, int E,
                  hipStream_t st);
int dropout_rows(float* x, long ld_n, long ld_t, const uint8_t* keep, long k_sn, long k_st, float scale, int N, int cnt,
                 int E, hipStream_t st);
int gather_words(const int64_t* src, long s_sn, long s_st, int64_t* dst, int N, int T, hipStream_t st);
int gru_fwd(const float* gi, long ld_gi, const float* gh, long ld_gh, const float* hp, long ld_hp, float* ho,
            long ld_ho, float* oseq, long ld_os, float* save, long ld_sv, float* hps, long ld_hps, const int64_t* lens,
            int t, int N, int H, hipStream_t st);
int gru_bwd(const float* dh_next, long ld_dn, const float* d_out, long ld_do, const float* save, long ld_sv,
            const float* hps, long ld_hps, float* dgi, long ld_dgi, float* dgh, long ld_dgh, float* dh_prev, long ld_dp,
            const int64_t* lens, int t, int N, int H, hipStream_t st);
int lstm_fwd(const float* gates, long ld_g, const float* cp, long ld_cp, float* ho, long ld_ho, float* co, long ld_co,
             float* save, long ld_sv, int N, int H, hipStream_t st);
int lstm_bwd(const float* dh, long ld_dh, const float* dc_next, long ld_dc, const float* save, long ld_sv,
             const float* cp, long ld_cp, float* dgates, long ld_dg, float* dc_prev, long ld_dcp, int N, int H,
             hipStream_t st);
int pool_fwd(const float* x, long ld_n, long ld_t, const int64_t* lens, float* out, int* argmax, int N, int T, int C,
             hipStream_t st);
int pool_bwd(const float* d, const int64_t* lens, const int* argmax, float* dx, long ld_n, long ld_t, int accumulate,
             int N, int T, int C, hipStream_t st);
int colsum_rows(const float* x, long ld, int rows, int cols, float* out, int accumulate, hipStream_t st);
int add_rows(float* dst, long ld_d, const float* src, long ld_s, int rows, int cols, hipStream_t st);
int copy_rows(float* dst, long ld_d, const float* src, long ld_s, int rows, int cols, hipStream_t st);
struct CopyRowsJob { float* dst; long ld_d; const float* src; long ld_s; int rows, cols; };
using CopyRowsBatch = JobTable<CopyRowsJob, 8>;
int copy_rows_batch(const CopyRowsBatch& b, hipStream_t st);
struct ZeroRegion { void* p; long words; };
struct ZeroBatch : JobTable<ZeroRegion, 16> {
  void add(void* p, long words) { if (p && words > 0) JobTable::add({p, words}); }
};
int zero_batch(const ZeroBatch& b, hipStream_t st);
}
```

### acvae_amd/csrc/rnn.hip

```cpp
#include "common.h"
#include "rnn.h"

namespace {

constexpr int TH = 256;
inline int grid1(long n) {
  long b = (n + TH - 1) / TH;
  return (int)(b < 1 ? 1 : (b > 4096 ? 4096 : b));
}

__global__ void caps_to_long_kernel(const float* __restrict__ caps, int64_t* __restrict__ out, long n) {
  for (long i = blockIdx.x * (long)TH + threadIdx.x; i < n; i += (long)gridDim.x * TH) out[i] = (int64_t)caps[i];
}
__global__ void select_word_kernel(const int64_t* __restrict__ caps, long ld_caps, const int64_t* __restrict__ seqs,
                                   long ld_seqs, int64_t* __restrict__ words, long ld_words, int t, int use_caps,
                                   int start_idx, int N) {
  const int n = blockIdx.x * TH + threadIdx.x;
  if (n >= N) return;
  int64_t w;
  if (use_caps) w = caps[n * ld_caps + t];
  else if (t == 0) w = start_idx;
  else w = seqs[n * ld_seqs + t - 1];
  words[n * ld_words + t] = w;
}
// ... 190 lines not shown
                                int accumulate, int N, int T, int C) {
  const long total = (long)N * T * C;
  for (long i = blockIdx.x * (long)TH + threadIdx.x; i < total; i += (long)gridDim.x * TH) {
    const int c = (int)(i % C);
    const int t = (int)((i / C) % T);
    const int n = (int)(i / ((long)C * T));
    const int len = (int)lens[n];
    float g = 0.f;
    if (t < len) {
      const float dv = d[n * C + c];
      g = dv / (float)len + (argmax[n * C + c] == t ? dv : 0.f);
    }
    float* p = dx + n * ld_n + t * ld_t + c;
    *p = accumulate ? *p + g : g;
  }
}

__global__ void colsum_rows_kernel(const float* __restrict__ x, long ld, int rows, int cols, float* __restrict__ out,
                                   int accumulate) {
  const int c = blockIdx.x * TH + threadIdx.x;
  if (c >= cols) return;
  float a = 0.f;
  for (int r = 0; r < rows; ++r) a += x[r * ld + c];
  out[c] = accumulate ? out[c] + a : a;
}
__global__ void add_rows_kernel(float* __restrict__ dst, long ld_d, const float* __restrict__ src, long ld_s, int rows,
                                int cols) {
  const long total = (long)rows * cols;
  for (long i = blockIdx.x * (long)TH + threadIdx.x; i < total; i += (long)gridDim.x * TH) {
    const int r = (int)(i / cols), c = (int)(i % cols);
    dst[r * ld_d + c] += src[r * ld_s + c];
  }
}
__global__ void copy_rows_kernel(float* __restrict__ dst, long ld_d, const float* __restrict__ src, long ld_s, int rows,
                                 int cols) {
  const long total = (long)rows * cols;
  for (long i = blockIdx.x * (long)TH + threadIdx.x; i < total; i += (long)gridDim.x * TH) {
    const int r = (int)(i / cols), c = (int)(i % cols);
    dst[r * ld_d + c] = src ? src[r * ld_s + c] : 0.f;
  }
}

__global__ void copy_rows_batch_kernel(acvae::CopyRowsBatch b) {
  const acvae::CopyRowsJob& j = b.job[blockIdx.y];
  const long total = (long)j.rows * j.cols;
  for (long i = blockIdx.x * (long)TH + threadIdx.x; i < total; i += (long)gridDim.x * TH) {
    const int r = (int)(i / j.cols), c = (int)(i % j.cols);
    j.dst[r * j.ld_d + c] = j.src ? j.src[r * j.ld_s + c] : 0.f;
  }
}

__global__ void zero_batch_kernel(acvae::ZeroBatch b) {
  unsigned* p = static_cast<unsigned*>(b.job[blockIdx.y].p);
  const long n = b.job[blockIdx.y].words;
  for (long i = blockIdx.x * (long)TH + threadIdx.x; i < n; i += (long)gridDim.x * TH) p[i] = 0u;
}

}

namespace acvae {
#define LAUNCH(k, g, ...) hipLaunchKernelGGL(k, dim3(g), dim3(TH), 0, st, __VA_ARGS__)
int zero_batch(const ZeroBatch& b, hipStream_t st) {
  if (!b.ok()) return ACVAE_EINVAL;
  if (b.n <= 0) return ACVAE_OK;
  long most = 1;
  for (int j = 0; j < b.n; ++j) if (b.job[j].words > most) most = b.job[j].words;
// ... 61 lines not shown
         ld_dgh, dh_prev, ld_dp, lens, t, N, H);
  ACVAE_LAUNCH_CHECK(); return ACVAE_OK;
}
int lstm_fwd(const float* gates, long ld_g, const float* cp, long ld_cp, float* ho, long ld_ho, float* co, long ld_co,
             float* save, long ld_sv, int N, int H, hipStream_t st) {
  LAUNCH(lstm_fwd_kernel, grid1((long)N * H), gates, ld_g, cp, ld_cp, ho, ld_ho, co, ld_co, save, ld_sv, N, H);
  ACVAE_LAUNCH_CHECK(); return ACVAE_OK;
}
int lstm_bwd(const float* dh, long ld_dh, const float* dc_next, long ld_dc, const float* save, long ld_sv,
             const float* cp, long ld_cp, float* dgates, long ld_dg, float* dc_prev, long ld_dcp, int N, int H,
             hipStream_t st) {
  LAUNCH(lstm_bwd_kernel, grid1((long)N * H), dh, ld_dh, dc_next, ld_dc, save, ld_sv, cp, ld_cp, dgates, ld_dg, dc_prev,
         ld_dcp, N, H);
  ACVAE_LAUNCH_CHECK(); return ACVAE_OK;
}
int pool_fwd(const float* x, long ld_n, long ld_t, const int64_t* lens, float* out, int* argmax, int N, int T, int C,
             hipStream_t st) {
  LAUNCH(pool_fwd_kernel, grid1((long)N * C), x, ld_n, ld_t, lens, out, argmax, N, T, C);
  ACVAE_LAUNCH_CHECK(); return ACVAE_OK;
}
int pool_bwd(const float* d, const int64_t* lens, const int* argmax, float* dx, long ld_n, long ld_t, int accumulate,
             int N, int T, int C, hipStream_t st) {
  LAUNCH(pool_bwd_kernel, grid1((long)N * T * C), d, lens, argmax, dx, ld_n, ld_t, accumulate, N, T, C);
  ACVAE_LAUNCH_CHECK(); return ACVAE_OK;
}
int colsum_rows(const float* x, long ld, int rows, int cols, float* out, int accumulate, hipStream_t st) {
  LAUNCH(colsum_rows_kernel, cdiv(cols, TH), x, ld, rows, cols, out, accumulate);
  ACVAE_LAUNCH_CHECK(); return ACVAE_OK;
}
int add_rows(float* dst, long ld_d, const float* src, long ld_s, int rows, int cols, hipStream_t st) {
  LAUNCH(add_rows_kernel, grid1((long)rows * cols), dst, ld_d, src, ld_s, rows, cols);
  ACVAE_LAUNCH_CHECK(); return ACVAE_OK;
}
int copy_rows(float* dst, long ld_d, const float* src, long ld_s, int rows, int cols, hipStream_t st) {
  LAUNCH(copy_rows_kernel, grid1((long)rows * cols), dst, ld_d, src, ld_s, rows, cols);
  ACVAE_LAUNCH_CHECK(); return ACVAE_OK;
}
#undef LAUNCH
}
```

### acvae_amd/streams.py

```python
import contextlib

import torch

_SCRATCH = {}


def scratch_buffer(nbytes, device, tag=None):
    key = (device.type, device.index, torch.cuda.current_stream(device).cuda_stream, tag)
    buf = _SCRATCH.get(key)
    if buf is None or buf.numel() < nbytes:
        _SCRATCH[key] = buf = torch.empty(int(nbytes), dtype=torch.uint8, device=device)
    return buf


def keep(stream, *objs, _seen=None):
    seen = set() if _seen is None else _seen
    for o in objs:
        if isinstance(o, (list, tuple, dict)):
            keep(stream, *(o.values() if isinstance(o, dict) else o), _seen=seen)
        elif getattr(o, "is_cuda", False) and id(o) not in seen:
            seen.add(id(o))
            o.record_stream(stream)


class SecondStreams:

    def __init__(self):
        self._made = {}

    def get(self, which, main):
        s = self._made.get(which)
        if s is None or s.device != main.device:
            s = self._made[which] = torch.cuda.Stream(device=main.device)
        return s

    def aux_handle(self):
        return self.get("decode", torch.cuda.current_stream()).cuda_stream


@contextlib.contextmanager
def beside(main, side, *inputs):
    results = []

    def on_side(fn, *args, **kw):
        with torch.cuda.stream(side):
# ... 24 lines not shown
```

### acvae_amd/train_util.py

```python
import numpy as np
import torch
import torch.nn as nn

from . import _lib


def _dev_scalar(dev):
    return torch.empty(1, device=dev)


class _CEFn(torch.autograd.Function):

    @staticmethod
    def forward(ctx, logits, targets, lens1, smoothing, reduction):
        _lib.require_cuda(logits)
        logits = logits.float()
        if not logits.is_contiguous():
            logits = logits.contiguous()
        N, T, V = logits.shape
        dev = logits.device
        targets = targets.to(device=dev, dtype=torch.long)
        if targets.stride(-1) != 1:
            targets = targets.contiguous()
        lens_d = None if lens1 is None else torch.as_tensor(lens1).to(device=dev, dtype=torch.long).contiguous()
# ... 112 lines not shown
    @staticmethod
    def backward(ctx, g):
        da = torch.empty_like(ctx.a) if ctx.needs_input_grad[0] else None
        db = torch.empty_like(ctx.b) if ctx.needs_input_grad[1] else None
        _lib.call("acvae_mse_bwd", ctx.a, ctx.b, g.contiguous().float().reshape(1), da, db, ctx.a.numel(),
                  _lib.current_stream())
        return da, db


class _CombineLossFn(torch.autograd.Function):

    @staticmethod
    def forward(ctx, ce, kl, mse, w_kl, w_mse):
        _lib.require_cuda(ce, kl)
        out = _dev_scalar(ce.device)
        _lib.call("acvae_loss_combine_fwd", ce.reshape(1), kl.reshape(1), None if mse is None else mse.reshape(1), float(w_kl),
                  float(w_mse), out, _lib.current_stream())
        ctx.w = (float(w_kl), float(w_mse), mse is not None)
        return out[0]

    @staticmethod
    def backward(ctx, g):
        w_kl, w_mse, has_mse = ctx.w
        gs = torch.empty(3, device=g.device)
        _lib.call("acvae_loss_combine_bwd", g.contiguous().float().reshape(1), w_kl, w_mse, gs[0:1], gs[1:2],
                  gs[2:3] if has_mse else None, _lib.current_stream())
        return gs[0], gs[1], (gs[2] if has_mse else None), None, None


def combine_losses(ce, kl, mse=None, kl_weight=1.0, alpha=0.0):
    return _CombineLossFn.apply(ce, kl, mse, kl_weight, alpha if mse is not None else 0.0)


class MSELoss(nn.Module):

    def forward(self, a, b):
        return _MSEFn.apply(a, b)


def _need_scorer(scorer):
    if scorer is None:
        raise ValueError("SCST needs a scorer: pass scorer=<object with compute_score(references, hypotheses) -> (score, "
                         "per-key scores)>, e.g. pycocoevalcap's Cider(), or acvae_amd.cider.CiderD(vocabulary), the package's own "
                         "CIDEr-D on the device")
    return scorer


def _on_device(scorer):
    from .cider import CiderD
    return isinstance(scorer, CiderD)


def _sentence(row, start_idx, end_idx, vocabulary):
    words = []
    for w_t in row:
        if w_t == start_idx:
            continue
        if w_t == end_idx:
            break
        words.append(vocabulary.idx2word[w_t])
    return " ".join(words)


def compute_batch_score(decode_res, key2refs, keys, start_idx, end_idx, vocabulary, scorer):
    scorer = _need_scorer(scorer)
    decode_res = np.asarray(decode_res)
# ... 145 lines not shown
```

### acvae_amd/trainer.py

```python
import contextlib
import math
import os

import numpy as np
import torch
import torch.distributed as dist

from . import _lib, streams
from .optim import FlatOptimizer, check_group, resolve
from .train_util import LabelSmoothingLoss, MSELoss, Normal_kl_loss, combine_losses


class FlatGradExchange:

    def __init__(self, flat, bucket_sizes, group=None, max_chunk=8 << 20):
        self.flat, self.group = flat, group
        self.world = dist.get_world_size(group) if dist.is_initialized() else 1
        self.max_chunk = int(max_chunk)
        self.slices, off = [], 0
        for n in bucket_sizes:
            self.slices.append((off, off + n))
            off += n
        assert off <= flat.numel()
        self._works, self._done, self.issued = [], set(), []
        self._xstream = None

    def begin(self):
        self._works, self._done, self.issued = [], set(), []

    def ready(self, i, after=()):
        if self.world == 1 or i in self._done:
            return
        self._done.add(i)
        a, b = self.slices[i]
        if b <= a:
            return
        ctx = contextlib.nullcontext()
        if self.flat.is_cuda:
            dev = self.flat.device
            produced = torch.cuda.Event()
            produced.record(torch.cuda.current_stream(dev))
            if self._xstream is None:
                self._xstream = torch.cuda.Stream(dev)
# ... 33 lines not shown
def _group_property(key):
    def get(self):
        return self.optimizer.param_groups[0].get(key)

    def set(self, value):
        self.optimizer.param_groups[0][key] = tuple(value) if key == "betas" else value
    return property(get, set, doc=f"optimizer.param_groups[0][{key!r}]")


class TrainStep:

    lr = _group_property("lr")
    betas = _group_property("betas")
    eps = _group_property("eps")
    weight_decay = _group_property("weight_decay")

    def __init__(self, model, vocab_size, lr=5e-4, betas=None, eps=None, weight_decay=None, max_grad_norm=1.0,
                 label_smoothing=True, smoothing=0.1, alpha=1.0, global_loss="MSE", process_group=None,
                 broadcast_buffers=True, data_parallel=True, precision=None, optimizer="Adam", optimizer_args=None):
        group = resolve(optimizer, optimizer_args, lr=lr, betas=betas, eps=eps, weight_decay=weight_decay)
        self.optimizer_name = optimizer
        self.model = model
        if precision is not None:
            model.encoder.compute_dtype = precision
        self.vocab = vocab_size
        self.max_grad_norm = max_grad_norm
        self.smoothing = smoothing if label_smoothing else 0.0
        self.alpha, self.global_loss = alpha, global_loss
        if alpha is not None and global_loss != "MSE":
            raise NotImplementedError("global_loss other than 'MSE' (the shipped q_logs_utt/p_logs_utt are None)")
        self.criterion = LabelSmoothingLoss(vocab_size, self.smoothing)
        self.kl_loss = Normal_kl_loss()
        self.mse_loss = MSELoss()
        self.pg = process_group
        self.data_parallel = data_parallel
        self.world = dist.get_world_size(process_group) if self._dist() else 1
        self.broadcast_buffers = broadcast_buffers
        self.step_count = 0
        self.max_steps_in_flight = int(os.environ.get("ACVAE_STEPS_IN_FLIGHT", "2"))
        self._in_flight = []
        self._copy_stream = None
        self._flatten(group)
        self.optimizer = FlatOptimizer(self, model.parameters(), optimizer, group)
        self._pending = None
        self.exchange = FlatGradExchange(self.flat_g, [self.n_text_dec, self.n_text - self.n_text_dec,
                                                       self.n_enc - self.n_enc_deep, self.n_enc_deep], process_group)
        if self.world == 1:
            self.exchange.world = 1
        if self.world > 1:
            model._grad_ready_cb = self._on_grads_ready
            model.encoder._grad_ready_cb = self._on_grads_ready
        self._buf_work = None
        self._decode_event = self._decode_aux_event = self._text_event = None
        self._decode_deferred = self._projemb_seen = False
        self._proj_emb = isinstance(model.decoder.word_embeddings, torch.nn.Sequential)
        if self.world > 1:
            join = lambda *_a, **_k: self.sync_buffers()
            model.register_forward_pre_hook(join)
            model.encoder.register_forward_pre_hook(join)
            model.register_state_dict_pre_hook(join)
        if self._dist():
            dist.broadcast(self.flat_p, src=0, group=self.pg)
            if self.flat_buf is not None:
                dist.broadcast(self.flat_buf, src=0, group=self.pg)

    def _dist(self):
# ... 65 lines not shown
        elif tag == "decode_deferred":
            self._decode_event, self._decode_aux_event = event
            self._decode_deferred = True
        elif tag == "projemb":
            self._projemb_seen = True
            if self._text_event is not None or not self._decode_deferred:
                self.exchange.ready(0, after=(self._decode_event, self._decode_aux_event, self._text_event))
        elif tag == "text":
            if torch.cuda.is_available() and self.flat_g.is_cuda:
                self._text_event = torch.cuda.Event()
                self._text_event.record(torch.cuda.current_stream())
            if not self._proj_emb or self._projemb_seen:
                self.exchange.ready(0, after=(self._decode_event, self._decode_aux_event))
            self.exchange.ready(1)
        elif isinstance(tag, tuple):
            if tag[1] == self.model.encoder._deep_block()[1]:
                self.exchange.ready(3)
        else:
            self.exchange.ready(3)
            self.exchange.ready(2)

    def forward_loss(self, feats, feat_lens, caps, cap_lens, ss_ratio=1.0, dis_ratio=0, kl_weight=0.5, clip_index=None,
                     frontend=None):
        if frontend is not None:
            feats, feat_lens = frontend(feats, feat_lens, device=self.flat_p.device)
        share = {} if clip_index is None else {"clip_index": clip_index}
        out = self.model(feats, feat_lens, caps, cap_lens, ss_ratio=ss_ratio, dis_ratio=dis_ratio, **share)
        staged = getattr(self.model, "staged", None) or {}
        lens1 = staged.get("lens1_d")
        if lens1 is None:
            lens1 = np.asarray(cap_lens) - 1
        caps_src = staged.get("caps_d")
        targets = (caps if caps_src is None else caps_src)[:, 1:1 + out["logits"].shape[1]].to(torch.long)
        ce = self.criterion.masked(out["logits"], targets, lens1)
        kl = self.kl_loss(out["q_means"], out["q_logs"], out["p_means"], out["p_logs"])
        mse = None
        if self.alpha is not None:
            mse = self.mse_loss(out["q_means_utt"], out["p_means_utt"])
        loss = combine_losses(ce, kl, mse, kl_weight, self.alpha if self.alpha is not None else 0.0)
        return loss, {"ce": ce.detach(), "kl": kl.detach(), "mse": None if mse is None else mse.detach()}, out

    def prefetch(self, feats_host):
        dev = self.flat_p.device
        t = torch.as_tensor(feats_host)
        if t.is_cuda:
            return t
        if self._copy_stream is None:
            self._copy_stream = torch.cuda.Stream(device=dev)
        with torch.cuda.stream(self._copy_stream):
            d = t.to(dev, non_blocking=True) if t.is_pinned() else _lib.h2d(t if t.dtype == torch.int16 else t.float(), dev)
            ev = torch.cuda.Event()
            ev.record(self._copy_stream)
        d._acvae_ready = ev
        return d

    def step(self, feats, feat_lens, caps, cap_lens, ss_ratio=1.0, dis_ratio=0, kl_weight=0.5, augment=None,
             clip_index=None, frontend=None):
        if frontend is not None:
            from .frontend import refuse_augment
            refuse_augment(augment)
        self.sync_buffers()
        ready = getattr(feats, "_acvae_ready", None)
        if ready is not None:
            streams.hand_over(feats, ready)
        if augment is not None:
            from .augment import apply
# ... 232 lines not shown
```

### acvae_amd/vae_model.py

```python
import contextlib
import os
import random
import weakref

import numpy as np
import torch
import torch.nn as nn

from . import _lib, search, streams, text_encoder
from .streams import scratch_buffer
from .word_model import CaptionModel
from .search import CONSTRAINTS_OFF, _constraint_args, length_norm


class _DecodeFn(torch.autograd.Function):
    @staticmethod
    def forward(ctx, model, mem, mem_lens_d, caps_d, lens1_d, q_z, eps_p, ss_flags, dis_flags, Tc, sampling, *weights):
        N, S, Eenc = mem.shape
        dec = model.decoder
        E, H, A, V = dec.embed_size, dec.model.hidden_size, dec.attn.attn_size, dec.vocab_size
        dev = mem.device
        train = caps_d is not None
        params = model._text_table()
        dims = (N, Tc, S, E, H, A, V, Eenc)
        saved_b = _lib.call("acvae_decode_saved_bytes", *dims)
        scratch_b = _lib.call("acvae_decode_scratch_bytes", *dims)
        if saved_b < 0:
            raise RuntimeError(f"decode: unsupported dims {dims}")
        saved = torch.empty(saved_b, dtype=torch.uint8, device=dev)
        scratch = scratch_buffer(scratch_b, dev)
        f = lambda *s: torch.empty(*s, device=dev)
        logits, outputs = f(N, Tc, V), f(N, Tc, H)
        seqs = torch.empty(N, Tc, dtype=torch.long, device=dev)
        slp, attw = f(N, Tc), f(N, Tc, S)
        pm, pl, pz = f(N, Tc, E), f(N, Tc, E), f(N, Tc, E)
        putt = f(N, 2 * E) if train else None
        hfin, hp, cp = f(N, H), f(N, E), f(N, E)
        IntArr = _lib.ctypes.c_int * Tc
        ss_arr = IntArr(*[int(bool(x)) for x in ss_flags]) if train else None
        dis_arr = IntArr(*[int(bool(x)) for x in dis_flags]) if train else IntArr(*([1] * Tc))
        mem = mem.contiguous()
        method, temp, noise = sampling["sample"] if sampling and sampling.get("sample") else (0, 1.0, None)
        keep, drop_p = sampling["emb_keep"] if sampling and sampling.get("emb_keep") else (None, 0.0)
        rollout = bool(not train and sampling and sampling.get("rollout_grad"))
        truncate = sampling.get("truncate") if sampling else None
        kept = torch.empty(N, Tc, dtype=torch.int32, device=dev) if truncate else None
        constrain = sampling.get("constrain") if sampling else None
        entry, extra = "acvae_decode_fwd_sampled", ()
        if truncate or constrain:
            entry = "acvae_decode_fwd_truncated"
            extra = (int(truncate[0]), float(truncate[1]), kept) if truncate else (0, 1.0, None)
        if constrain:
            entry, extra = "acvae_decode_fwd_constrained", extra + search._constraint_args(constrain)
        _lib.persist_status(dev)
        _lib.call(entry, params, mem,
                  mem_lens_d, caps_d, caps_d.stride(0) if train else 0, lens1_d, q_z, eps_p, ss_arr, dis_arr, logits,
                  outputs, seqs, slp, attw, pm, pl, pz, putt, hfin, hp, cp, saved, saved_b, scratch, scratch_b, *dims, model.start_idx,
                  model.end_idx, _lib.current_stream(), model._aux_stream(), int(method), float(temp), noise, keep,
                  float(drop_p), _lib.call_flags() | (_lib.FLAG_ROLLOUT_GRAD if rollout else 0), *extra)
        ctx.set_materialize_grads(False)
        ctx.model, ctx.saved, ctx.dims, ctx.dis_arr = model, saved, dims, dis_arr
        ctx.emb_keep, ctx.emb_p, ctx.rollout = keep, float(drop_p), rollout
        ctx.save_for_backward(mem, mem_lens_d, lens1_d, eps_p, outputs, attw, pl, *((logits, seqs) if rollout else ()))
        ctx.mark_non_differentiable(seqs, attw, hfin, hp, cp, *(() if rollout else (slp,)))
        if not train:
            putt = torch.zeros(0, device=dev)
            ctx.mark_non_differentiable(putt)
        if kept is not None:
            ctx.mark_non_differentiable(kept)
            return logits, outputs, seqs, slp, attw, pm, pl, pz, putt, hfin, hp, cp, kept
        return logits, outputs, seqs, slp, attw, pm, pl, pz, putt, hfin, hp, cp

    @staticmethod
    def backward(ctx, d_logits, d_outputs, _s, d_slp, _a, d_pm, d_pl, d_pz, d_putt, *_rest):
        model = ctx.model
        N, Tc, S, E, H, A, V, Eenc = ctx.dims
        mem, mem_lens_d, lens1_d, eps_p, outputs, attw, pl = ctx.saved_tensors[:7]
        dev = mem.device
        params = model._text_table()
        grads = [None] * len(params)
        mine = set(range(0, 10)) | set(range(21, 35))
        if ctx.rollout:
            mine -= {31, 32}
            if d_slp is not None:
                logits, seqs = ctx.saved_tensors[7:]
                off = _lib.call("acvae_decode_saved_lse_offset", *ctx.dims)
                lse = ctx.saved[off:off + N * Tc * 4].view(torch.float32)
                dl = torch.empty(N, Tc, V, device=dev)
                _lib.call("acvae_logprob_bwd", logits, V, lse, seqs, d_slp.contiguous().float(), dl, N * Tc, V,
                          _lib.current_stream())
                d_logits = dl if d_logits is None else dl.add_(d_logits)
        for i, p in enumerate(params):
# ... 242 lines not shown
            feats, feat_lens, caps, cap_lens = input
            if self.decoder.model.hidden_size != self.decoder.embed_size:
                raise ValueError(f"training forward: the decoder's hidden_size ({self.decoder.model.hidden_size}) must equal "
                                 f"its embed_size ({self.decoder.embed_size}); other hidden sizes decode only (the "
                                 "2-input forward, beam search, rollouts)")
            share = None if clip_index is None else clip_rows(clip_index, len(feat_lens), len(cap_lens))
            if share is not None and feats.shape[0] != len(feat_lens):
                raise ValueError(f"clip_index: {feats.shape[0]} feature rows for {len(feat_lens)} feature lengths")
            n_rows = feats.shape[0] if share is None else len(cap_lens)
            main = torch.cuda.current_stream()
            side = self.streams.get("posterior", main) if self.use_side_stream else main
            eps_q = None if self.noise is None else self.noise.get("eps_q")
            q_keep = None if self.noise is None else self.noise.get("q_keep")
            lens1 = np.asarray(cap_lens) - 1
            q_p = self.qnet.keep_p()
            if q_p > 0:
                q, Tc = self.qnet, int(lens1.max())
                if q_keep is None:
                    q_keep = _lib.h2d_fill((q.num_layers - 1, n_rows, Tc, 2 * q.hidden_size), torch.uint8,
                                           feats.device, lambda buf: text_encoder.posterior_keep_masks(
                                               lens1, Tc, q.hidden_size, q.num_layers, q_p, out=buf))
                else:
                    q_keep = _lib.h2d(q_keep, feats.device, torch.uint8).contiguous()
            if eps_q is None:
                eps_q = torch.randn(n_rows, int(lens1.max()), self.decoder.embed_size)
            prep = self._host_prepare(n_rows, feats.device, caps, cap_lens, kwargs)
            if share is not None:
                share = (share[0],) + tuple(_lib.h2d(a, feats.device) for a in share[:3])
            with streams.beside(main, side, prep["caps_d"], q_keep) as on_side:
                encoded = self.encoder(feats, feat_lens) if encoder_output is None else encoder_output
                if share is not None:
                    encoded = self._share_rows(encoded, *share)
                qnetout = on_side(self.qnet, prep["caps_d"], cap_lens, eps=eps_q, keep=q_keep)
            encoded["_prep"] = prep
            encoded.update(qnetout)
            return self.train_forward(encoded, caps, cap_lens, **kwargs)
        if len(input) == 2:
            feats, feat_lens = input
            encoded = self.encoder(feats, feat_lens)
            return self.inference_forward(encoded, **kwargs)
        raise Exception("Number of input should be either 4 (feats, feat_lens, caps, cap_lens) or 2 (feats, feat_lens)")

    def _share_rows(self, encoded, index, index_d, offsets_d, rows_d):
        mem, pooled = encoded["audio_embeds"], encoded["audio_embeds_pooled"].detach().contiguous()
        B, N = mem.shape[0], index_d.shape[0]
        pooled_rows = torch.empty(N, pooled.shape[1], device=pooled.device)
        _lib.call("acvae_rows_gather", pooled, index_d, pooled_rows, B, N, pooled.shape[1], _lib.current_stream())
        lens = torch.as_tensor(encoded["audio_embeds_lens"])[torch.from_numpy(index)]
        return {"audio_embeds": _ShareRowsFn.apply(mem, index_d, offsets_d, rows_d), "audio_embeds_pooled": pooled_rows,
                "state": None, "audio_embeds_lens": lens, "audio_embeds_lens_dev": _lib.h2d(lens, mem.device, torch.long)}

    def rollout_shared_encoder(self, feats, feat_lens, sample_n, **kwargs):
        rerank = kwargs.pop("rerank", None)
        self._rerank_check(rerank, sample_n, kwargs)
        self._truncation(kwargs, rollout=True)
        self._constraints(kwargs, rollout=True)
        self._forward_token = getattr(self, "_forward_token", 0) + 1
        encoded = self.encoder(feats, feat_lens)
        n = int(sample_n)
        lens = torch.as_tensor(np.asarray(encoded["audio_embeds_lens"])).repeat_interleave(n, dim=0)
        rep = {"audio_embeds": encoded["audio_embeds"].repeat_interleave(n, dim=0),
               "audio_embeds_pooled": encoded["audio_embeds_pooled"].repeat_interleave(n, dim=0),
               "audio_embeds_lens": lens, "state": None}
        return self._rerank(self.inference_forward(rep, **kwargs), rerank, n)

    def _rerank_check(self, rerank, sample_n, kwargs):
        search.rerank_check(rerank, sample_n, kwargs, self.max_length, self._records_rollout())

    def _rerank(self, output, rerank, sample_n):
        if rerank is None:
            return output
        got = rerank.select(output["seqs"], sample_n, int(self.start_idx), int(self.end_idx))
        output["candidates"] = output["seqs"]
        output["seqs"] = got["seqs"]
# ... 78 lines not shown
            sampling["sample"] = (code, temp, noise_d)
        elif code:
            if sample_noise is None:
                sample_noise = torch.as_tensor(replay["sample_noise"])[:Tc]
            sampling["sample"] = (code, temp, _lib.h2d(sample_noise, dev, torch.float32).contiguous())
        if top_k > 0 or top_p < 1.0:
            sampling["truncate"] = (top_k, top_p)
        if constrain != search.CONSTRAINTS_OFF:
            sampling["constrain"] = constrain
        if drop_p > 0.0:
            if dec_keep is None:
                dec_keep = torch.as_tensor(replay["dec_keep"])[:Tc]
            sampling["emb_keep"] = (_lib.h2d(dec_keep.to(torch.uint8), dev).contiguous(), drop_p)
        return {"Tc": Tc, "ss_flags": ss_flags, "dis_flags": dis_flags, "eps_p": eps_p, "caps_d": caps_d,
                "lens1_d": lens1_d, "sampling": sampling}

    def stepwise_forward(self, encoded, caps, cap_lens, **kwargs):
        mem = encoded["audio_embeds"]
        dev = mem.device
        N = mem.shape[0]
        E = self.decoder.embed_size
        train = caps is not None
        mem_lens_d = encoded.get("audio_embeds_lens_dev")
        if mem_lens_d is None:
            mem_lens_d = _lib.h2d(encoded["audio_embeds_lens"], dev, torch.long)
        prep = encoded.pop("_prep", None) or self._host_prepare(N, dev, caps, cap_lens, kwargs)
        record = train or self._records_rollout()
        if record and not train:
            prep["sampling"] = dict(prep.get("sampling") or {}, rollout_grad=True)
        Tc, ss_flags, dis_flags, eps_p = prep["Tc"], prep["ss_flags"], prep["dis_flags"], prep["eps_p"]
        caps_d, lens1_d = prep["caps_d"], prep["lens1_d"]
        q_z = encoded["q_z"] if train else None
        self.staged = {"caps_d": caps_d, "lens1_d": lens1_d}
        with contextlib.nullcontext() if record else torch.no_grad():
            outs = _DecodeFn.apply(self, mem, mem_lens_d, caps_d, lens1_d, q_z, eps_p, ss_flags, dis_flags, Tc,
                                   prep.get("sampling"), *self._decode_weights())
        logits, outputs, seqs, slp, attw, pm, pl, pz, putt, hfin, hp, cp = outs[:12]
        output = {"seqs": seqs, "logits": logits, "outputs": outputs, "sampled_logprobs": slp,
                  "attn_weights": attw.transpose(1, 2), "p_means": pm, "p_logs": pl, "p_z": pz,
                  "state": hfin.unsqueeze(0), "hiddens_state": (hp.unsqueeze(0), cp.unsqueeze(0)), "last_z": pz[:, -1]}
        if len(outs) > 12:
            output["kept"] = outs[12]
        if train:
            for k in ("q_means", "q_logs", "q_z", "q_means_utt", "q_logs_utt"):
                output[k] = encoded[k]
            output["p_means_utt"] = putt
            output["p_logs_utt"] = None
        return output
```

### include/acvae_hip.h

```cpp
#ifndef ACVAE_HIP_H
#define ACVAE_HIP_H
#include <stdint.h>
#ifdef __cplusplus
extern "C" {
#endif

#define ACVAE_ABI_VERSION 3
int acvae_abi_version(void);

#define ACVAE_FLAG_NO_PERSIST 1
#define ACVAE_FLAG_DEFER_PARAM_GRADS 2
#define ACVAE_FLAG_NO_ATTN_SPLIT 4
#define ACVAE_FLAG_ROLLOUT_GRAD 16
#define ACVAE_FLAG_TEST_STALL 8

int acvae_persist_status_register(int device, void* status_words_host);

int acvae_gemm_nt(const float* A, int64_t lda, const float* B, int64_t ldb, const float* bias, float* C,
                  int64_t ldc, int M, int N, int K, int accumulate, void* stream);
int acvae_gemm_tn(const float* A, int64_t lda, const float* B, int64_t ldb, float* C, int64_t ldc, int M, int N,
                  int K, int accumulate, float* slab_ws, int64_t slab_ws_bytes, void* stream);
int64_t acvae_gemm_tn_workspace_bytes(int M, int N, int K);
int64_t acvae_colsum_workspace_bytes(int cols);
int acvae_colsum(const float* x, int rows, int cols, float* out, void* ws, int64_t ws_bytes, void* stream);

int64_t acvae_gemm_nt_splitk_workspace_bytes(void);
int acvae_gemm_nt_split_plan(int M, int N, int K1, int K2, int with_ws);
int acvae_gemm_nt_dual_ws(const float* A1, int64_t lda1, const float* B1, int64_t ldb1, int K1, const float* A2,
                          int64_t lda2, const float* B2, int64_t ldb2, int K2, const float* bias, float* C, int64_t ldc,
                          int M, int N, int accumulate, float* ws, int64_t ws_bytes, int reset_tickets, void* stream);
int acvae_gemm_nt_pair_c(const float* A0, int64_t lda0, const float* B0, int64_t ldb0, int K0, const float* bias0, float* C0,
                         int64_t ldc0, int N0, int acc0, const float* A1, int64_t lda1, const float* B1, int64_t ldb1, int K1,
                         const float* bias1, float* C1, int64_t ldc1, int N1, int acc1, int M, void* stream);
int64_t acvae_gemm_tn_fused_workspace_bytes(int M, int N, int K);
int acvae_gemm_tn_fused_plan(int M, int N, int K, int64_t ws_bytes);
int acvae_gemm_tn_fused_c(const float* A, int64_t lda, const float* B, int64_t ldb, float* C, int64_t ldc, int M, int N,
                          int K, int accumulate, float* ws, int64_t ws_bytes, int reset_tickets, void* stream);
int64_t acvae_gemm_tn_group_workspace_bytes(int n, const int* M, const int* N, const int* K);
int acvae_gemm_tn_group_c(int n, const void* const* A, const int64_t* lda, const void* const* B, const int64_t* ldb,
                          const void* const* C, const int64_t* ldc, const int* M, const int* N, const int* K, void* ws,
                          int64_t ws_bytes, int reset_tickets, void* stream);
int64_t acvae_colsum_batch_workspace_bytes(int n, const int* P, const int* width);
int acvae_colsum_batch_plan(int n, const int* P, const int* width, int64_t ws_bytes);
int acvae_colsum_batch(int n, const void* const* x, const int* P, const int* width, const void* const* out,
                       const void* const* out_b, void* ws, int64_t ws_bytes, int reset_tickets, void* stream);
int acvae_transpose(const float* in, int64_t ld_in, float* out, int64_t ld_out, int rows, int cols, void* stream);

int64_t acvae_attn_fwd_workspace_bytes(int N, int Tq, int S, int A, int E);
int acvae_attn_fwd(const float* qproj, int64_t q_sn, int64_t q_sj, const float* encproj, const float* enc,
                   const int64_t* lens, const float* v, float* ctx, int64_t c_sn, int64_t c_sj, float* weights,
                   int64_t w_sn, int64_t w_sj, int N, int Tq, int S, int A, int E, void* ws, int64_t ws_bytes, void* stream,
                   int flags);
int acvae_tanh_att(const float* x, float* y, int64_t n, void* stream);
int64_t acvae_attn_bwd_workspace_bytes(int N, int Tq, int S, int A);
int acvae_attn_bwd(const float* dctx, int64_t dc_sn, int64_t dc_sj, const float* qproj, int64_t q_sn, int64_t q_sj,
                   const float* encproj, const float* enc, const int64_t* lens, const float* v,
                   const float* weights, int64_t w_sn, int64_t w_sj, float* dqproj, int64_t dq_sn, int64_t dq_sj,
                   float* dencproj, float* denc, float* dv_part, float* ws, int64_t ws_bytes, int N, int Tq, int S,
                   int A, int E, void* stream);

int acvae_reparam_fwd(const float* ml, int64_t ld_ml, const float* eps, int64_t ld_eps, float* mean, float* logv,
                      float* z, int64_t ld_out, float* z2, int64_t ld_z2, int rows, int E, void* stream);
int acvae_reparam_bwd(const float* dz, int64_t ld_dz, const float* dmean_ext, const float* dlog_ext, int64_t ld_ext,
// ... 24 lines not shown
                    float* out_scalar, int N, int T, int V, void* stream);
int acvae_ls_ce_bwd(const float* logits, int64_t ld_n, int64_t ld_t, const int64_t* targets, int64_t tg_sn,
                    const int64_t* lens1, const float* lse, float smoothing, int reduction, const float* grad_out,
                    const float* grad_rows, float* dlogits, int N, int T, int V, void* stream);
int acvae_scst_loss_fwd(const float* sampled_logprobs, const int64_t* seqs, const float* reward, int end_idx, float* coef,
                        float* loss, int N, int Tc, void* stream);
int acvae_logprob_bwd(const float* logits, int64_t ld, const float* lse, const int64_t* seqs, const float* coef,
                      float* d_logits, int64_t rows, int V, void* stream);
#define ACVAE_CIDER_MAX_LENGTH 64
int acvae_ciderd_scores(const int64_t* seqs0, const int64_t* seqs1, int64_t ld, int n, int n_sets, int max_length,
                        int start_idx, int end_idx, const uint64_t* idf_keys, const double* idf_vals, int n_idf,
                        double log_d, const uint64_t* ref_keys, const double* ref_w, int n_entries, const int* ref_off,
                        const double* ref_norm, const int* ref_len, int n_refs, const int* doc_ref, int n_docs,
                        const int* row_doc, const int* row_src, const double* len_factor, int n_len, double* score,
                        void* stream);
int acvae_ciderd_reward(const double* score, int n, int sample_n, float* reward, double* reward_mean, void* stream);
#define ACVAE_CONSENSUS_MAX_LENGTH 64
#define ACVAE_CONSENSUS_MAX_SAMPLES 16
int acvae_consensus_scores(const int64_t* seqs, int64_t ld, int n, int sample_n, int max_length, int start_idx, int end_idx,
                           const uint64_t* idf_keys, const double* idf_vals, int n_idf, double log_d,
                           const double* len_factor, int n_len, double* score, int64_t* best, int64_t* picked, void* stream);
#define ACVAE_DIVERSITY_HEAD 5
#define ACVAE_DIVERSITY_PER_CANDIDATE 6
int acvae_diversity_stats(const int64_t* seqs, int64_t ld, int n, int sample_n, int max_length, int start_idx, int end_idx,
                          int V, int* record, int* seen, void* stream);
#define ACVAE_ACCURACY_RECORD 9
int acvae_accuracy_stats(const int64_t* seqs, int64_t ld, int n, int sample_n, int max_length, int start_idx, int end_idx,
                         int V, const int* ref_words, int n_words, const int* ref_off, int n_refs, const int* clip_ref,
                         int n_clips, int* record, void* stream);
int acvae_mse_fwd(const float* a, const float* b, float* partials, float* out_scalar, int64_t n, void* stream);
int acvae_mse_bwd(const float* a, const float* b, const float* grad_out, float* da, float* db, int64_t n, void* stream);
int acvae_loss_combine_fwd(const float* ce, const float* kl, const float* mse, float w_kl, float w_mse, float* out, void* stream);
int acvae_loss_combine_bwd(const float* grad_out, float w_kl, float w_mse, float* g_ce, float* g_kl, float* g_mse, void* stream);

#define ACVAE_ENC_NPARAMS 55
#define ACVAE_ARCH_CNN10 0
#define ACVAE_ARCH_CNN14_16K 1
#define ACVAE_ARCH_RESNET38 2
#define ACVAE_ENC_BF16 256
int acvae_encoder_nparams(int arch);
int acvae_encoder_out_dims(int arch, int T, int* S, int* C);
int64_t acvae_encoder_saved_bytes(int arch, int N, int T, int F);
int64_t acvae_encoder_scratch_bytes(int arch, int N, int T, int F);
int acvae_encoder_fwd(const void* const* params, const float* feats, float* audio_embeds, float* pooled,
                      void* saved, int64_t saved_bytes, void* scratch, int64_t scratch_bytes, int arch, int N, int T,
                      int F, int training, float p_block, float p_fc, uint64_t seed, const uint8_t* const* masks,
                      void* stream);
int acvae_encoder_bwd(const void* const* params, void* const* grads, const float* feats,
                      const float* d_audio_embeds, void* saved, int64_t saved_bytes, void* scratch,
                      int64_t scratch_bytes, int arch, int N, int T, int F, int training, float p_block, uint64_t seed,
                      const uint8_t* const* masks, void* stream);
int acvae_encoder_relu_mask(const void* saved, int64_t saved_bytes, int arch, int N, int T, int F, int site,
                            uint8_t* mask_nchw, void* stream);
int acvae_encoder_bwd_hooked(const void* const* params, void* const* grads, const float* feats,
                             const float* d_audio_embeds, void* saved, int64_t saved_bytes, void* scratch,
                             int64_t scratch_bytes, int arch, int N, int T, int F, int training, float p_block,
                             uint64_t seed, const uint8_t* const* masks, void* stream, void* block_done, void* user);

int64_t acvae_conv3x3_workspace_bytes(int N, int H, int W, int Cin, int Cout);
int acvae_conv3x3_fwd(const float* X, const float* W_oihw, const float* in_scale, const float* in_shift, float* Y,
                      const float* gamma, const float* beta, float* running_mean, float* running_var,
                      int64_t* num_batches_tracked, int training, float* bn_out, void* ws, int64_t ws_bytes, int N, int H,
                      int W, int Cin, int Cout, void* stream);
int acvae_conv3x3_dgrad(const float* dY, const float* W_oihw, float* dX, void* ws, int64_t ws_bytes, int N, int H, int W,
                        int Cin, int Cout, void* stream);
int acvae_conv3x3_wgrad(const float* dY, const float* X, const float* in_scale, const float* in_shift, float* dW_oihw,
// ... 78 lines not shown
                        const float* eps_q, float* q_means, float* q_logs, float* q_z, float* q_means_utt,
                        void* saved, int64_t saved_bytes, void* scratch, int64_t scratch_bytes, int N, int Tc, int E,
                        int Hq, int V, void* stream, int flags);
int acvae_posterior_bwd(const void* const* params, void* const* grads, const int64_t* lens1, const float* eps_q,
                        const float* q_logs, const float* d_q_means, const float* d_q_logs, const float* d_q_z,
                        const float* d_q_means_utt, void* saved, int64_t saved_bytes, void* scratch,
                        int64_t scratch_bytes, int N, int Tc, int E, int Hq, int V, void* stream, int flags);

int64_t acvae_posterior_stack_saved_bytes(int N, int Tc, int E, int Hq, int V, int num_layers);
int64_t acvae_posterior_stack_scratch_bytes(int N, int Tc, int E, int Hq, int V, int num_layers);
int acvae_posterior_stack_fwd(const void* const* params, const void* const* upper, int num_layers, const uint8_t* keep,
                              float keep_scale, const int64_t* caps, int64_t ld_caps, const int64_t* lens1,
                              const float* eps_q, float* q_means, float* q_logs, float* q_z, float* q_means_utt,
                              void* saved, int64_t saved_bytes, void* scratch, int64_t scratch_bytes, int N, int Tc,
                              int E, int Hq, int V, void* stream, int flags);
int acvae_posterior_stack_bwd(const void* const* params, void* const* grads, const void* const* upper,
                              void* const* upper_grads, int num_layers, const uint8_t* keep, float keep_scale,
                              const int64_t* lens1, const float* eps_q, const float* q_logs, const float* d_q_means,
                              const float* d_q_logs, const float* d_q_z, const float* d_q_means_utt, void* saved,
                              int64_t saved_bytes, void* scratch, int64_t scratch_bytes, int N, int Tc, int E, int Hq,
                              int V, void* stream, int flags);


int64_t acvae_decode_saved_bytes(int N, int Tc, int S, int E, int H, int A, int V, int Eenc);
int64_t acvae_decode_scratch_bytes(int N, int Tc, int S, int E, int H, int A, int V, int Eenc);
int64_t acvae_decode_saved_lse_offset(int N, int Tc, int S, int E, int H, int A, int V, int Eenc);
int acvae_decode_fwd(const void* const* params, const float* mem_in, const int64_t* mem_lens, const int64_t* caps,
                     int64_t ld_caps, const int64_t* lens1, const float* q_z, const float* eps_p,
                     const int* ss_flags_host, const int* dis_flags_host, float* logits, float* outputs, int64_t* seqs,
                     float* sampled_logprobs, float* attn_w, float* p_means, float* p_logs, float* p_z,
                     float* p_means_utt, float* h_final, float* hp_final, float* cp_final, void* saved,
                     int64_t saved_bytes, void* scratch, int64_t scratch_bytes, int N, int Tc, int S, int E, int H,
                     int A, int V, int Eenc, int start_idx, int end_idx, void* stream, void* aux_stream, int flags);
int acvae_decode_fwd_sampled(const void* const* params, const float* mem_in, const int64_t* mem_lens,
                             const int64_t* caps, int64_t ld_caps, const int64_t* lens1, const float* q_z,
                             const float* eps_p, const int* ss_flags_host, const int* dis_flags_host, float* logits,
                             float* outputs, int64_t* seqs, float* sampled_logprobs, float* attn_w, float* p_means,
                             float* p_logs, float* p_z, float* p_means_utt, float* h_final, float* hp_final,
                             float* cp_final, void* saved, int64_t saved_bytes, void* scratch, int64_t scratch_bytes,
                             int N, int Tc, int S, int E, int H, int A, int V, int Eenc, int start_idx, int end_idx,
                             void* stream, void* aux_stream, int sample_method, float temp, const float* sample_noise,
                             const uint8_t* emb_keep, float emb_drop_p, int flags);
int acvae_decode_fwd_truncated(const void* const* params, const float* mem_in, const int64_t* mem_lens,
                               const int64_t* caps, int64_t ld_caps, const int64_t* lens1, const float* q_z,
                               const float* eps_p, const int* ss_flags_host, const int* dis_flags_host, float* logits,
                               float* outputs, int64_t* seqs, float* sampled_logprobs, float* attn_w, float* p_means,
                               float* p_logs, float* p_z, float* p_means_utt, float* h_final, float* hp_final,
                               float* cp_final, void* saved, int64_t saved_bytes, void* scratch, int64_t scratch_bytes,
                               int N, int Tc, int S, int E, int H, int A, int V, int Eenc, int start_idx, int end_idx,
                               void* stream, void* aux_stream, int sample_method, float temp, const float* sample_noise,
                               const uint8_t* emb_keep, float emb_drop_p, int flags, int top_k, float top_p,
                               int32_t* kept);
int acvae_decode_bwd_defers(const int* dis_flags_host, int Tc, void* stream, void* aux_stream, int flags);
int acvae_decode_bwd(const void* const* params, void* const* grads, const float* mem_in, const int64_t* mem_lens,
                     const int64_t* lens1, const float* eps_p, const int* dis_flags_host, const float* outputs,
                     const float* attn_w, const float* p_logs, const float* d_logits, const float* d_outputs_ext,
                     const float* d_p_means, const float* d_p_logs, const float* d_p_z, const float* d_p_means_utt,
                     float* d_mem_in, float* d_q_z, void* saved, int64_t saved_bytes, void* scratch,
                     int64_t scratch_bytes, int N, int Tc, int S, int E, int H, int A, int V, int Eenc, void* stream,
                     void* aux_stream, const uint8_t* emb_keep, float emb_drop_p, int flags);
int acvae_caps_to_long(const float* caps, int64_t* out, int64_t n, void* stream);

int64_t acvae_grad_norm_partials(void);
int acvae_grad_norm(const float* grads, int64_t n, float grad_scale, float* partials, float* out_norm, void* stream);
int acvae_adam_step(float* params, const float* grads, float* exp_avg, float* exp_avg_sq, int64_t n, float lr,
                    float beta1, float beta2, float eps, float weight_decay, int64_t step, float grad_scale,
// ... 160 lines not shown
```

Baseline: 2145.

## Precompute decoder input projections on aux stream and reorder backward for overlap

Adds a decode_fwd_pre entry point that gathers words, embeds, and computes the prior attention query and decoder input-gate GEMMs on an auxiliary stream right after the posterior, so the main decode forward can skip them with a PRE_DONE flag. The backward pass is reordered: decoder dz is computed early and written directly into d_q_z, the prior input-gradient GEMM is split in two halves so attention backward can start sooner, and the dmem sum is written straight into d_mem_in without an extra copy. It also adds a fused VAE loss (CE+KL+MSE) using the saved log-sum-exp from decode. An OLD_ORDER flag keeps the previous schedule available. These changes add stream synchronisation and extra memory, and the reordering widens what can go wrong.

```diff
diff --git a/acvae_amd/_lib.py b/acvae_amd/_lib.py
--- a/acvae_amd/_lib.py
+++ b/acvae_amd/_lib.py
@@ -61,6 +61,8 @@
 FLAG_NO_ATTN_SPLIT = int(_defs["ACVAE_FLAG_NO_ATTN_SPLIT"])
 FLAG_TEST_STALL = int(_defs["ACVAE_FLAG_TEST_STALL"])
 FLAG_ROLLOUT_GRAD = int(_defs["ACVAE_FLAG_ROLLOUT_GRAD"])
+FLAG_OLD_ORDER = int(_defs["ACVAE_FLAG_OLD_ORDER"])
+FLAG_PRE_DONE = int(_defs["ACVAE_FLAG_PRE_DONE"])
 _lib = None
 
 
@@ -69,6 +71,7 @@
     defer = os.environ.get("ACVAE_DECODE_DEFER", "1") != "0"
     attn_split = True
     test_stall = False
+    old_order = False
 
 
 class override:
@@ -110,6 +113,8 @@
         f |= FLAG_NO_ATTN_SPLIT
     if options.test_stall:
         f |= FLAG_TEST_STALL
+    if options.old_order:
+        f |= FLAG_OLD_ORDER
     if defer and options.defer:
         f |= FLAG_DEFER_PARAM_GRADS
     return f
diff --git a/acvae_amd/csrc/conv.h b/acvae_amd/csrc/conv.h
--- a/acvae_amd/csrc/conv.h
+++ b/acvae_amd/csrc/conv.h
@@ -107,7 +107,7 @@
 
 int acvae_gemm_nt_dual(const float* A1, int64_t lda1, const float* B1, int64_t ldb1, int K1, const float* A2,
                        int64_t lda2, const float* B2, int64_t ldb2, int K2, const float* bias, float* C, int64_t ldc,
-                       int M, int N, int accumulate, hipStream_t st, float* skws = nullptr);
+                       int M, int N, int accumulate, hipStream_t st, float* skws = nullptr, int plan_N = 0);
 int acvae_gemm_nt_pair(const float* A0, int64_t lda0, const float* B0, int64_t ldb0, int K0, const float* bias0, float* C0,
                        int64_t ldc0, int N0, int acc0, const float* A1, int64_t lda1, const float* B1, int64_t ldb1, int K1,
                        const float* bias1, float* C1, int64_t ldc1, int N1, int acc1, int M, hipStream_t st);
diff --git a/acvae_amd/csrc/decoder.hip b/acvae_amd/csrc/decoder.hip
--- a/acvae_amd/csrc/decoder.hip
+++ b/acvae_amd/csrc/decoder.hip
@@ -582,6 +582,8 @@
   acvae::PdPlan pd_plan{};
   const bool persist_fwd = teacher && !prior_feeds_decoder && !(flags & ACVAE_FLAG_NO_PERSIST) && H == E &&
                            acvae::decode_fwd_resident(N, Tc, S, E, H, A, pd_plan);
+  const bool pre_done = (flags & ACVAE_FLAG_PRE_DONE) != 0;
+  if (pre_done && !(teacher && !prior_feeds_decoder)) return ACVAE_EINVAL;
   const bool attws_ready = !persist_fwd && L.attfws_bytes > 0;
   {
     acvae::ZeroBatch zb;
@@ -621,10 +623,12 @@
   auto ldof = [&](int cnt, long C) { return cnt == Tc ? C : (long)Tc * C; };
   auto prior_pre = [&](int t0, int cnt) -> int {
     const int M = rows_of(cnt);
-    ACVAE_TRY(acvae::embed_gather(words + t0, cnt == Tc ? 1 : Tc, P(TP_P_EMB), V, rnn_p + (long)t0 * 3 * E,
-                                  ldof(cnt, 3 * E), M, E, sp));
-    ACVAE_TRY(gemm(rnn_p + (long)t0 * 3 * E, ldof(cnt, 3 * E), P(TP_P_ATT_W), 2 * E, nullptr, qp + (long)t0 * E,
-                   ldof(cnt, E), M, E, E, 0, sp));
+    if (!pre_done) {
+      ACVAE_TRY(acvae::embed_gather(words + t0, cnt == Tc ? 1 : Tc, P(TP_P_EMB), V, rnn_p + (long)t0 * 3 * E,
+                                    ldof(cnt, 3 * E), M, E, sp));
+      ACVAE_TRY(gemm(rnn_p + (long)t0 * 3 * E, ldof(cnt, 3 * E), P(TP_P_ATT_W), 2 * E, nullptr, qp + (long)t0 * E,
+                     ldof(cnt, E), M, E, E, 0, sp));
+    }
     ACVAE_TRY(acvae_attn_fwd(qp + (long)t0 * E, (long)Tc * E, E, encproj_p, mem, mem_lens, P(TP_P_ATT_V),
                              rnn_p + (long)t0 * 3 * E + E, ld3E, 3 * E, attw_p + (long)t0 * S, (long)Tc * S, S, N, cnt, S,
                              E, E, (cnt == 1 && attws_ready) ? sc + L.attfws_p : nullptr, L.attfws_bytes, sp, flags));
@@ -653,6 +657,7 @@
     return ACVAE_OK;
   };
   auto dec_pre = [&](int t0, int cnt) -> int {
+    if (pre_done) return ACVAE_OK;
     const int M = rows_of(cnt);
     ACVAE_TRY(acvae::embed_gather(words + t0, cnt == Tc ? 1 : Tc, P(TP_DEC_EMB), V, rnn_d + (long)t0 * 3 * E,
                                   ldof(cnt, 3 * E), M, E, st));
@@ -730,7 +735,7 @@
   };
 
   if (teacher) {
-    ACVAE_TRY(acvae::gather_words(caps, ld_caps, 1, words, N, Tc, st));
+    if (!pre_done) ACVAE_TRY(acvae::gather_words(caps, ld_caps, 1, words, N, Tc, st));
     ACVAE_TRY(fork.begin());
     ACVAE_TRY(encproj_prior(sp));
     ACVAE_TRY(encproj_dec());
@@ -854,6 +859,38 @@
                            top_k, top_p, kept, con);
 }
 
+extern "C" int acvae_decode_fwd_pre(const void* const* params, const int64_t* caps, int64_t ld_caps, const float* q_z,
+                                    void* saved_v, int64_t saved_bytes, void* scratch_v, int64_t scratch_bytes, int N, int Tc,
+                                    int S, int E, int H, int A, int V, int Eenc, void* stream, const uint8_t* emb_keep,
+                                    float emb_drop_p, int flags) {
+  (void)flags;
+  if (emb_keep && !(emb_drop_p > 0.f && emb_drop_p <= 1.f)) return ACVAE_EINVAL;
+  DecLayout L;
+  ACVAE_TRY(dec_layout(N, Tc, S, E, H, A, V, Eenc, L));
+  if (!params || !caps || !q_z || !saved_v || !scratch_v) return ACVAE_EINVAL;
+  if (H != E) return ACVAE_EUNSUPPORTED;
+  if (saved_bytes < L.saved_total * 4 || scratch_bytes < dec_scratch_floats(L) * 4) return ACVAE_EWORKSPACE;
+  float* sv = (float*)saved_v;
+  float* sc = (float*)scratch_v;
+  auto P = [&](int i) { return (const float*)params[i]; };
+  const int R = N * Tc;
+  const Ctx c{(hipStream_t)stream, sc + L.skws_p};
+  ACVAE_TRY(acvae_skinny_ws_reset(c.skws, c.s));
+  int64_t* words = (int64_t*)(sv + L.words);
+  float* rnn_d = sv + L.rnn_d;
+  float* rnn_p = sv + L.rnn_p;
+  ACVAE_TRY(acvae::gather_words(caps, ld_caps, 1, words, N, Tc, c));
+  ACVAE_TRY(acvae::embed_gather(words, 1, P(TP_P_EMB), V, rnn_p, 3 * E, R, E, c));
+  ACVAE_TRY(gemm(rnn_p, 3 * E, P(TP_P_ATT_W), 2 * E, nullptr, sv + L.qp, E, R, E, E, 0, c));
+  ACVAE_TRY(acvae::embed_gather(words, 1, P(TP_DEC_EMB), V, rnn_d, 3 * E, R, E, c));
+  if (emb_keep)
+    ACVAE_TRY(acvae::dropout_rows(rnn_d, (long)Tc * 3 * E, 3 * E, emb_keep, E, (long)N * E,
+                                  emb_drop_p < 1.f ? 1.f / (1.f - emb_drop_p) : 0.f, N, Tc, E, c));
+  ACVAE_TRY(acvae::copy_rows(rnn_d + 2 * E, 3 * E, q_z, E, R, E, c));
+  return gemm2(rnn_d, 3 * E, P(TP_DEC_WIH), 3 * E, E, rnn_d + 2 * E, 3 * E, P(TP_DEC_WIH) + 2 * E, 3 * E, E, P(TP_DEC_BIH),
+               sc + L.gi_d, 3 * H, R, 3 * H, 0, c);
+}
+
 extern "C" int acvae_decode_bwd_defers(const int* dis_flags_host, int Tc, void* stream, void* aux_stream, int flags) {
   if (!(flags & ACVAE_FLAG_DEFER_PARAM_GRADS) || !aux_stream || aux_stream == stream || !dis_flags_host) return 0;
   for (int t = 0; t < Tc; ++t)
@@ -896,6 +933,7 @@
   const int R = N * Tc, Hp = E;
   const bool defer = acvae_decode_bwd_defers(dis_flags_host, Tc, stream, aux_stream, flags) != 0;
   const bool has_ln = Eenc != E || params[TP_LN_W] != nullptr;
+  const bool old_order = (flags & ACVAE_FLAG_OLD_ORDER) != 0;
   TnWs tn{sc + L.tn, L.tn_floats * 4};
   TnWs tn_p{sc + L.tn_p, L.tn_p_floats * 4};
   double* dpart = (double*)(sc + L.dpart);
@@ -999,6 +1037,8 @@
     return gemm(dencproj, A, wt_datt + (long)H * A, A, nullptr, dmem, E, N * S, E, A, 1, st);
   };
   auto dec_dz = [&](const Ctx& c) -> int {
+    if (d_q_z && !prior_feeds_decoder && !old_order)
+      return gemm(dgi, 3 * H, wt_dih + (long)2 * E * 3 * H, 3 * H, nullptr, d_q_z, E, R, E, 3 * H, 0, c);
     ACVAE_TRY(gemm(dgi, 3 * H, wt_dih + (long)2 * E * 3 * H, 3 * H, nullptr, dz_dec, E, R, E, 3 * H, 0, c));
     if (!d_q_z) return ACVAE_OK;
     if (!prior_feeds_decoder) {
@@ -1086,7 +1126,11 @@
   };
   float* dqp = sc + L.dqp;
   auto prior_memgrad = [&]() -> int {
-    ACVAE_TRY(gemm(dgates, 4 * Hp, wt_pih, 4 * Hp, nullptr, drnn_p, 3 * E, R, 2 * E, 4 * Hp, 0, sp));
+    if (old_order)
+      ACVAE_TRY(gemm(dgates, 4 * Hp, wt_pih, 4 * Hp, nullptr, drnn_p, 3 * E, R, 2 * E, 4 * Hp, 0, sp));
+    else
+      ACVAE_TRY(acvae_gemm_nt_dual(dgates, 4 * Hp, wt_pih + (long)E * 4 * Hp, 4 * Hp, 4 * Hp, nullptr, 0, nullptr, 0, 0, nullptr,
+                                   drnn_p + E, 3 * E, R, E, 0, sp.s, sp.skws, 2 * E));
     ACVAE_TRY(zero(dencproj_p, (long)N * S * E, sp));
     ACVAE_TRY(zero(dvpart_p, (long)N * E, sp));
     ACVAE_TRY(acvae_attn_bwd(drnn_p + E, (long)Tc * 3 * E, 3 * E, sv + L.qp, (long)Tc * E, E, sv + L.encproj_p, mem,
@@ -1113,10 +1157,14 @@
       cb.add({dencproj_p, N * S, E, G(TP_P_ATT_B)}); cb.add({dvpart_p, N, E, G(TP_P_ATT_V)});
       ACVAE_TRY(acvae::colsum_batch(cb, dpart_p, L.dpart_doubles, sp));
     }
+    if (!old_order)
+      ACVAE_TRY(acvae_gemm_nt_dual(dgates, 4 * Hp, wt_pih, 4 * Hp, 4 * Hp, nullptr, 0, nullptr, 0, 0, nullptr, drnn_p, 3 * E, R,
+                                   E, 0, sp.s, sp.skws, 2 * E));
     ACVAE_TRY(gemm(dqp, E, wt_patt, E, nullptr, drnn_p, 3 * E, R, E, E, 1, sp));
     return acvae::embed_scatter(words_c, drnn_p, 3 * E, G(TP_P_EMB), V, R, E, sp);
   };
   bool early_tn = false;
+  bool dz_early = false;
   if (prior_feeds_decoder) {
     ACVAE_TRY(dec_begin());
     for (int t = Tc - 1; t >= 0; --t) ACVAE_TRY(dec_bptt(t));
@@ -1142,8 +1190,11 @@
     pb.dqd_part = sc + L.pd_dqd; pb.ctx = rnn_d + E;
     ACVAE_TRY(acvae::decode_persist_bwd(pb, pb_plan, st.s, flags));
     dv_rows = pb_plan.dv_rows;
-    ACVAE_TRY(dec_memgrad());
+    if (old_order) ACVAE_TRY(dec_memgrad());
     if (fork.on()) ACVAE_TRY(Fork::edge(st.s, sp.s));
+    if (!old_order) ACVAE_TRY(dec_memgrad());
+    dz_early = defer && !old_order;
+    if (dz_early) ACVAE_TRY(dec_dz(st));
     ACVAE_TRY(prior_memgrad());
     if (!defer) {
       ACVAE_TRY(dec_params(st, tn, dpart));
@@ -1170,17 +1221,18 @@
     }
   }
   ACVAE_TRY(fork.join());
-  ACVAE_TRY(acvae::add_rows(dmem, E, dmem_p, E, N * S, E, st));
+  if (has_ln || old_order) ACVAE_TRY(acvae::add_rows(dmem, E, dmem_p, E, N * S, E, st));
+  else ACVAE_TRY(acvae::add_rows(d_mem_in, E, dmem, E, dmem_p, E, N * S, E, st));
   if (has_ln) {
     ACVAE_TRY(transp(P(TP_LN_W), Eenc, wt_ln, E, E, Eenc, st));
     ACVAE_TRY(gemm(dmem, E, wt_ln, E, nullptr, d_mem_in, Eenc, N * S, Eenc, E, 0, st));
     ACVAE_TRY(gemm_tn(dmem, E, mem_in, Eenc, G(TP_LN_W), Eenc, E, Eenc, N * S, tn, st));
     ACVAE_TRY(acvae::colsum2(dmem, N * S, E, dpart, G(TP_LN_B), nullptr, 0, st));
-  } else {
+  } else if (old_order) {
     ACVAE_TRY(acvae::copy_rows(d_mem_in, E, dmem, E, N * S, E, st));
   }
   if (defer) {
-    ACVAE_TRY(dec_dz(st));
+    if (!dz_early) ACVAE_TRY(dec_dz(st));
     ACVAE_TRY(Fork::edge(st.s, sp.s));
     ACVAE_TRY(dec_params(sp, tn_p, dpart_p, false, !early_tn));
     ACVAE_TRY(prior_params(!early_tn));
diff --git a/acvae_amd/csrc/gemm.hip b/acvae_amd/csrc/gemm.hip
--- a/acvae_amd/csrc/gemm.hip
+++ b/acvae_amd/csrc/gemm.hip
@@ -331,12 +331,14 @@
 
 int acvae_gemm_nt_dual(const float* A1, int64_t lda1, const float* B1, int64_t ldb1, int K1, const float* A2,
                        int64_t lda2, const float* B2, int64_t ldb2, int K2, const float* bias, float* C, int64_t ldc,
-                       int M, int N, int accumulate, hipStream_t st, float* skws) {
+                       int M, int N, int accumulate, hipStream_t st, float* skws, int plan_N) {
   if (!A1 || !B1 || !C || M <= 0 || N <= 0 || K1 <= 0) return ACVAE_EINVAL;
   if (A2 && (!B2 || K2 <= 0)) return ACVAE_EINVAL;
+  if (plan_N && plan_N < N) return ACVAE_EINVAL;
+  if (!plan_N) plan_N = N;
   bool vec = vec_ok(A1, lda1, K1) && vec_ok(B1, ldb1, K1);
   if (A2) vec = vec && vec_ok(A2, lda2, K2) && vec_ok(B2, ldb2, K2);
-  const int S = skinny_plan(M, N, K1 + (A2 ? K2 : 0), A2 != nullptr, skws != nullptr);
+  const int S = skinny_plan(M, plan_N, K1 + (A2 ? K2 : 0), A2 != nullptr, skws != nullptr);
   if (S > 0) {
     dim3 grid(cdiv(N, 32), cdiv(M, 32), S);
     unsigned* cnt = (unsigned*)skws;
@@ -350,7 +352,7 @@
     ACVAE_LAUNCH_CHECK();
     return ACVAE_OK;
   }
-  const bool bn64 = (N <= 64);
+  const bool bn64 = (plan_N <= 64);
   dim3 grid(cdiv(M, 128), cdiv(N, bn64 ? 64 : 128));
 #define LAUNCH_NT(BN_, V_)                                                                                     \
   hipLaunchKernelGGL((gemm_nt_kernel<BN_, V_>), grid, dim3(nt_threads<128>()), 0, st, A1, lda1, B1, ldb1, bias, C, ldc, M, \
@@ -514,6 +516,15 @@
   if (ws && reset_tickets) ACVAE_TRY(acvae_skinny_ws_reset(ws, st));
   return acvae_gemm_nt_dual(A1, lda1, B1, ldb1, K1, A2, lda2, B2, ldb2, K2, bias, C, ldc, M, N, accumulate, st, ws);
 }
+extern "C" int acvae_gemm_nt_cols_ws(const float* A, int64_t lda, const float* B, int64_t ldb, int K, const float* bias, float* C,
+                                     int64_t ldc, int M, int N, int plan_N, int accumulate, float* ws, int64_t ws_bytes,
+                                     int reset_tickets, void* stream) {
+  if (!A || !B || !C || M <= 0 || N <= 0 || K <= 0 || plan_N < N) return ACVAE_EINVAL;
+  if (ws && ws_bytes < acvae_gemm_nt_splitk_workspace_bytes()) return ACVAE_EWORKSPACE;
+  hipStream_t st = (hipStream_t)stream;
+  if (ws && reset_tickets) ACVAE_TRY(acvae_skinny_ws_reset(ws, st));
+  return acvae_gemm_nt_dual(A, lda, B, ldb, K, nullptr, 0, nullptr, 0, 0, bias, C, ldc, M, N, accumulate, st, ws, plan_N);
+}
 extern "C" int acvae_gemm_nt_pair_c(const float* A0, int64_t lda0, const float* B0, int64_t ldb0, int K0, const float* bias0,
                                     float* C0, int64_t ldc0, int N0, int acc0, const float* A1, int64_t lda1, const float* B1,
                                     int64_t ldb1, int K1, const float* bias1, float* C1, int64_t ldc1, int N1, int acc1, int M,
diff --git a/acvae_amd/csrc/losses.hip b/acvae_amd/csrc/losses.hip
--- a/acvae_amd/csrc/losses.hip
+++ b/acvae_amd/csrc/losses.hip
@@ -1,5 +1,6 @@
 #include "common.h"
 #include "dbs_rules.h"
+#include "job_table.h"
 #include "../../include/acvae_hip.h"
 
 namespace {
@@ -39,7 +40,7 @@
   }
 }
 
-__global__ void final_sum_kernel(const float* __restrict__ partials, int n, float scale, float* __restrict__ out) {
+__device__ __forceinline__ void final_sum_body(const float* __restrict__ partials, int n, float scale, float* __restrict__ out) {
   __shared__ float red[16];
   double acc = 0.0;
   for (int i = threadIdx.x; i < n; i += blockDim.x) acc += (double)partials[i];
@@ -54,38 +55,46 @@
   }
   (void)red;
 }
+__global__ void final_sum_kernel(const float* __restrict__ partials, int n, float scale, float* __restrict__ out) {
+  final_sum_body(partials, n, scale, out);
+}
 
 __device__ __forceinline__ float kl_elem(float mu1, float lv1, float mu2, float lv2) {
   const float d = mu1 - mu2;
   return lv2 * .5f - lv1 * .5f + (expf(lv1) + d * d) / (2.f * expf(lv2)) - .5f;
 }
 
+__device__ __forceinline__ void kl_fwd_body(const float* __restrict__ mu1, const float* __restrict__ lv1,
+                                            const float* __restrict__ mu2, const float* __restrict__ lv2,
+                                            float* __restrict__ partials, long n, int bid, int nb) {
+  __shared__ float red[16];
+  float acc = 0.f;
+  const long n4 = n >> 2;
+  for (long i = bid * (long)EW_THREADS + threadIdx.x; i < n4; i += (long)nb * EW_THREADS) {
+    const float4 a = reinterpret_cast<const float4*>(mu1)[i], b = reinterpret_cast<const float4*>(lv1)[i];
+    const float4 c = reinterpret_cast<const float4*>(mu2)[i], d = reinterpret_cast<const float4*>(lv2)[i];
+    acc += kl_elem(a.x, b.x, c.x, d.x) + kl_elem(a.y, b.y, c.y, d.y) + kl_elem(a.z, b.z, c.z, d.z) +
+           kl_elem(a.w, b.w, c.w, d.w);
+  }
+  if (bid == 0)
+    for (long i = (n4 << 2) + threadIdx.x; i < n; i += EW_THREADS) acc += kl_elem(mu1[i], lv1[i], mu2[i], lv2[i]);
+  acc = block_sum(acc, red);
+  if (threadIdx.x == 0) partials[bid] = acc;
+}
 __global__ __launch_bounds__(EW_THREADS) void kl_fwd_kernel(const float* __restrict__ mu1,
                                                             const float* __restrict__ lv1,
                                                             const float* __restrict__ mu2,
                                                             const float* __restrict__ lv2, float* __restrict__ partials,
                                                             long n) {
-  __shared__ float red[16];
-  float acc = 0.f;
-  const long n4 = n >> 2;
-  for (long i = blockIdx.x * (long)EW_THREADS + threadIdx.x; i < n4; i += (long)gridDim.x * EW_THREADS) {
-    const float4 a = reinterpret_cast<const float4*>(mu1)[i], b = reinterpret_cast<const float4*>(lv1)[i];
-    const float4 c = reinterpret_cast<const float4*>(mu2)[i], d = reinterpret_cast<const float4*>(lv2)[i];
-    acc += kl_elem(a.x, b.x, c.x, d.x) + kl_elem(a.y, b.y, c.y, d.y) + kl_elem(a.z, b.z, c.z, d.z) +
-           kl_elem(a.w, b.w, c.w, d.w);
-  }
-  if (blockIdx.x == 0)
-    for (long i = (n4 << 2) + threadIdx.x; i < n; i += EW_THREADS) acc += kl_elem(mu1[i], lv1[i], mu2[i], lv2[i]);
-  acc = block_sum(acc, red);
-  if (threadIdx.x == 0) partials[blockIdx.x] = acc;
-}
-
-__global__ void kl_bwd_kernel(const float* __restrict__ mu1, const float* __restrict__ lv1,
-                              const float* __restrict__ mu2, const float* __restrict__ lv2,
-                              const float* __restrict__ grad_out, float inv_rows, float* __restrict__ dmu1,
-                              float* __restrict__ dlv1, float* __restrict__ dmu2, float* __restrict__ dlv2, long n) {
-  const float g = grad_out[0] * inv_rows;
-  for (long i = blockIdx.x * (long)blockDim.x + threadIdx.x; i < n; i += (long)gridDim.x * blockDim.x) {
+  kl_fwd_body(mu1, lv1, mu2, lv2, partials, n, (int)blockIdx.x, (int)gridDim.x);
+}
+
+__device__ __forceinline__ void kl_bwd_body(const float* __restrict__ mu1, const float* __restrict__ lv1,
+                                            const float* __restrict__ mu2, const float* __restrict__ lv2, float g0,
+                                            float inv_rows, float* __restrict__ dmu1, float* __restrict__ dlv1,
+                                            float* __restrict__ dmu2, float* __restrict__ dlv2, long n, int bid, int nb) {
+  const float g = g0 * inv_rows;
+  for (long i = bid * (long)blockDim.x + threadIdx.x; i < n; i += (long)nb * blockDim.x) {
     const float d = mu1[i] - mu2[i];
     const float v1 = expf(lv1[i]), iv2 = 1.f / expf(lv2[i]);
     if (dmu1) dmu1[i] = g * d * iv2;
@@ -94,27 +103,41 @@
     if (dlv2) dlv2[i] = g * (.5f - .5f * (v1 + d * d) * iv2);
   }
 }
-
+__global__ void kl_bwd_kernel(const float* __restrict__ mu1, const float* __restrict__ lv1,
+                              const float* __restrict__ mu2, const float* __restrict__ lv2,
+                              const float* __restrict__ grad_out, float inv_rows, float* __restrict__ dmu1,
+                              float* __restrict__ dlv1, float* __restrict__ dmu2, float* __restrict__ dlv2, long n) {
+  kl_bwd_body(mu1, lv1, mu2, lv2, grad_out[0], inv_rows, dmu1, dlv1, dmu2, dlv2, n, (int)blockIdx.x, (int)gridDim.x);
+}
+
+__device__ __forceinline__ void mse_fwd_body(const float* __restrict__ a, const float* __restrict__ b,
+                                             float* __restrict__ partials, long n, int bid, int nb) {
+  __shared__ float red[16];
+  float acc = 0.f;
+  for (long i = bid * (long)EW_THREADS + threadIdx.x; i < n; i += (long)nb * EW_THREADS) {
+    const float d = a[i] - b[i];
+    acc += d * d;
+  }
+  acc = block_sum(acc, red);
+  if (threadIdx.x == 0) partials[bid] = acc;
+}
 __global__ __launch_bounds__(EW_THREADS) void mse_fwd_kernel(const float* __restrict__ a, const float* __restrict__ b,
                                                              float* __restrict__ partials, long n) {
-  __shared__ float red[16];
-  float acc = 0.f;
-  for (long i = blockIdx.x * (long)EW_THREADS + threadIdx.x; i < n; i += (long)gridDim.x * EW_THREADS) {
-    const float d = a[i] - b[i];
-    acc += d * d;
-  }
-  acc = block_sum(acc, red);
-  if (threadIdx.x == 0) partials[blockIdx.x] = acc;
+  mse_fwd_body(a, b, partials, n, (int)blockIdx.x, (int)gridDim.x);
+}
+__device__ __forceinline__ void mse_bwd_body(const float* __restrict__ a, const float* __restrict__ b, float g0, float scale,
+                                             float* __restrict__ da, float* __restrict__ db, long n, int bid, int nb) {
+  const float g = g0 * scale;
+  for (long i = bid * (long)blockDim.x + threadIdx.x; i < n; i += (long)nb * blockDim.x) {
+    const float d = g * (a[i] - b[i]);
+    if (da) da[i] = d;
+    if (db) db[i] = -d;
+  }
 }
 __global__ void mse_bwd_kernel(const float* __restrict__ a, const float* __restrict__ b,
                                const float* __restrict__ grad_out, float scale, float* __restrict__ da,
                                float* __restrict__ db, long n) {
-  const float g = grad_out[0] * scale;
-  for (long i = blockIdx.x * (long)blockDim.x + threadIdx.x; i < n; i += (long)gridDim.x * blockDim.x) {
-    const float d = g * (a[i] - b[i]);
-    if (da) da[i] = d;
-    if (db) db[i] = -d;
-  }
+  mse_bwd_body(a, b, grad_out[0], scale, da, db, n, (int)blockIdx.x, (int)gridDim.x);
 }
 
 __global__ __launch_bounds__(EW_THREADS) void row_stats_kernel(const float* __restrict__ logits, long ld_n, long ld_t,
@@ -361,13 +384,12 @@
   }
 }
 
-__global__ __launch_bounds__(EW_THREADS) void ce_rows_kernel(const float* __restrict__ logits, long ld_n, long ld_t,
-                                                             const int64_t* __restrict__ targets, long tg_sn,
-                                                             const int64_t* __restrict__ lens1,
-                                                             const float* __restrict__ lse, float smoothing,
-                                                             float* __restrict__ loss_rows, int T, int V) {
+__device__ __forceinline__ void ce_rows_body(const float* __restrict__ logits, long ld_n, long ld_t,
+                                             const int64_t* __restrict__ targets, long tg_sn,
+                                             const int64_t* __restrict__ lens1, const float* __restrict__ lse,
+                                             float smoothing, float* __restrict__ loss_rows, int T, int V, int bid) {
   __shared__ float red[16];
-  const int n = blockIdx.x / T, t = blockIdx.x % T;
+  const int n = bid / T, t = bid % T;
   const long o = (long)n * T + t;
   if (lens1 && t >= (int)lens1[n]) {
     if (threadIdx.x == 0) loss_rows[o] = 0.f;
@@ -385,9 +407,16 @@
     loss_rows[o] = -((1.f - smoothing) * lpt + (smoothing != 0.f ? smoothing / (float)(V - 1) * (sumlp - lpt) : 0.f));
   }
 }
-
-__global__ void ce_reduce_kernel(const float* __restrict__ loss_rows, const int64_t* __restrict__ lens1, int N, int T,
-                                 int mean, float* __restrict__ out) {
+__global__ __launch_bounds__(EW_THREADS) void ce_rows_kernel(const float* __restrict__ logits, long ld_n, long ld_t,
+                                                             const int64_t* __restrict__ targets, long tg_sn,
+                                                             const int64_t* __restrict__ lens1,
+                                                             const float* __restrict__ lse, float smoothing,
+                                                             float* __restrict__ loss_rows, int T, int V) {
+  ce_rows_body(logits, ld_n, ld_t, targets, tg_sn, lens1, lse, smoothing, loss_rows, T, V, (int)blockIdx.x);
+}
+
+__device__ __forceinline__ void ce_reduce_body(const float* __restrict__ loss_rows, const int64_t* __restrict__ lens1, int N,
+                                               int T, int mean, float* __restrict__ out) {
   __shared__ double redd[16];
   double acc = 0.0;
   for (int i = threadIdx.x; i < N * T; i += blockDim.x) acc += (double)loss_rows[i];
@@ -405,7 +434,39 @@
     out[0] = (float)t;
   }
 }
-
+__global__ void ce_reduce_kernel(const float* __restrict__ loss_rows, const int64_t* __restrict__ lens1, int N, int T,
+                                 int mean, float* __restrict__ out) {
+  ce_reduce_body(loss_rows, lens1, N, T, mean, out);
+}
+
+__device__ __forceinline__ void ce_bwd_body(const float* __restrict__ logits, long ld_n, long ld_t,
+                                            const int64_t* __restrict__ targets, long tg_sn,
+                                            const int64_t* __restrict__ lens1, const float* __restrict__ lse,
+                                            float smoothing, int reduction, float g0, const float* __restrict__ grad_rows,
+                                            float* __restrict__ dlogits, int N, int T, int V, int bid) {
+  const int n = bid / T, t = bid % T;
+  float* d = dlogits + n * ld_n + t * ld_t;
+  if (lens1 && t >= (int)lens1[n]) {
+    for (int c = threadIdx.x; c < V; c += EW_THREADS) d[c] = 0.f;
+    return;
+  }
+  float g;
+  if (reduction == 0) {
+    g = grad_rows[(long)n * T + t];
+  } else {
+    g = g0;
+    if (reduction == 1) {
+      long cnt = 0;
+      for (int i = 0; i < N; ++i) cnt += lens1 ? (lens1[i] < T ? lens1[i] : T) : T;
+      g /= (float)cnt;
+    }
+  }
+  const float* x = logits + n * ld_n + t * ld_t;
+  const float l = lse[(long)n * T + t];
+  const int tg = (int)targets[n * tg_sn + t];
+  const float off = smoothing / (float)(V - 1), on = 1.f - smoothing;
+  for (int c = threadIdx.x; c < V; c += EW_THREADS) d[c] = g * (expf(x[c] - l) - (c == tg ? on : off));
+}
 __global__ __launch_bounds__(EW_THREADS) void ce_bwd_kernel(const float* __restrict__ logits, long ld_n, long ld_t,
                                                             const int64_t* __restrict__ targets, long tg_sn,
                                                             const int64_t* __restrict__ lens1,
@@ -413,28 +474,8 @@
                                                             int reduction, const float* __restrict__ grad_out,
                                                             const float* __restrict__ grad_rows,
                                                             float* __restrict__ dlogits, int N, int T, int V) {
-  const int n = blockIdx.x / T, t = blockIdx.x % T;
-  float* d = dlogits + n * ld_n + t * ld_t;
-  if (lens1 && t >= (int)lens1[n]) {
-    for (int c = threadIdx.x; c < V; c += EW_THREADS) d[c] = 0.f;
-    return;
-  }
-  float g;
-  if (reduction == 0) {
-    g = grad_rows[(long)n * T + t];
-  } else {
-    g = grad_out[0];
-    if (reduction == 1) {
-      long cnt = 0;
-      for (int i = 0; i < N; ++i) cnt += lens1 ? (lens1[i] < T ? lens1[i] : T) : T;
-      g /= (float)cnt;
-    }
-  }
-  const float* x = logits + n * ld_n + t * ld_t;
-  const float l = lse[(long)n * T + t];
-  const int tg = (int)targets[n * tg_sn + t];
-  const float off = smoothing / (float)(V - 1), on = 1.f - smoothing;
-  for (int c = threadIdx.x; c < V; c += EW_THREADS) d[c] = g * (expf(x[c] - l) - (c == tg ? on : off));
+  ce_bwd_body(logits, ld_n, ld_t, targets, tg_sn, lens1, lse, smoothing, reduction, reduction != 0 ? grad_out[0] : 0.f,
+              grad_rows, dlogits, N, T, V, (int)blockIdx.x);
 }
 
 __global__ __launch_bounds__(EW_THREADS) void scst_loss_kernel(const float* __restrict__ slp,
@@ -731,6 +772,108 @@
   return ACVAE_OK;
 }
 
+namespace {
+enum { VL_CE, VL_KL, VL_MSE };
+struct VlJob { int kind; };
+using VlTable = acvae::RangeTable<VlJob, 3, int>;
+struct VlArgs {
+  const float* logits; long ld_n, ld_t; const int64_t* targets; long tg_sn; const int64_t* lens1; const float* lse;
+  float smoothing; float* loss_rows; int N, T, V;
+  const float *mu1, *lv1, *mu2, *lv2; long kl_n, kl_rows; float* kl_part;
+  const float *a, *b; long mse_n; float* mse_part;
+  float w_kl, w_mse;
+  const float* grad_out; float *dlogits, *dmu1, *dlv1, *dmu2, *dlv2, *da, *db;
+};
+__global__ __launch_bounds__(EW_THREADS) void vae_loss_rows_kernel(VlTable tb, VlArgs p) {
+  const int l = tb.find((int)blockIdx.x);
+  const int bid = (int)blockIdx.x - tb.start[l], nb = tb.start[l + 1] - tb.start[l];
+  switch (tb.job[l].kind) {
+    case VL_CE: ce_rows_body(p.logits, p.ld_n, p.ld_t, p.targets, p.tg_sn, p.lens1, p.lse, p.smoothing, p.loss_rows, p.T, p.V, bid); break;
+    case VL_KL: kl_fwd_body(p.mu1, p.lv1, p.mu2, p.lv2, p.kl_part, p.kl_n, bid, nb); break;
+    default: mse_fwd_body(p.a, p.b, p.mse_part, p.mse_n, bid, nb); break;
+  }
+}
+__global__ __launch_bounds__(256) void vae_loss_final_kernel(VlArgs p, int kl_nb, int mse_nb, float* __restrict__ out) {
+  ce_reduce_body(p.loss_rows, p.lens1, p.N, p.T, 1, out + 1);
+  __syncthreads();
+  final_sum_body(p.kl_part, kl_nb, (float)(1.0 / (double)p.kl_rows), out + 2);
+  __syncthreads();
+  final_sum_body(p.mse_part, mse_nb, (float)(1.0 / (double)p.mse_n), out + 3);
+  if (threadIdx.x == 0) {
+    float v = out[1] + p.w_kl * out[2];
+    v = v + p.w_mse * out[3];
+    out[0] = v;
+  }
+}
+__global__ __launch_bounds__(EW_THREADS) void vae_loss_bwd_kernel(VlTable tb, VlArgs p) {
+  const int l = tb.find((int)blockIdx.x);
+  const int bid = (int)blockIdx.x - tb.start[l], nb = tb.start[l + 1] - tb.start[l];
+  const float v = p.grad_out[0];
+  switch (tb.job[l].kind) {
+    case VL_CE:
+      ce_bwd_body(p.logits, p.ld_n, p.ld_t, p.targets, p.tg_sn, p.lens1, p.lse, p.smoothing, 1, v, nullptr, p.dlogits, p.N, p.T,
+                  p.V, bid);
+      break;
+    case VL_KL:
+      kl_bwd_body(p.mu1, p.lv1, p.mu2, p.lv2, v * p.w_kl, (float)(1.0 / (double)p.kl_rows), p.dmu1, p.dlv1, p.dmu2, p.dlv2,
+                  p.kl_n, bid, nb);
+      break;
+    default: mse_bwd_body(p.a, p.b, v * p.w_mse, (float)(2.0 / (double)p.mse_n), p.da, p.db, p.mse_n, bid, nb); break;
+  }
+}
+}
+static int vl_check(const float* logits, const int64_t* targets, const float* lse, const float* mu1, const float* lv1,
+                    const float* mu2, const float* lv2, int64_t kl_rows, int E, const float* a, const float* b, int64_t mse_n, int N,
+                    int T, int V) {
+  if (!logits || !targets || !lse || N <= 0 || T <= 0 || V <= 1) return ACVAE_EINVAL;
+  if (!mu1 || !lv1 || !mu2 || !lv2 || kl_rows <= 0 || E <= 0 || !a || !b || mse_n <= 0) return ACVAE_EINVAL;
+  if (!aligned16(mu1) || !aligned16(lv1) || !aligned16(mu2) || !aligned16(lv2)) return ACVAE_EALIGN;
+  return ACVAE_OK;
+}
+extern "C" int acvae_vae_loss_fwd(const float* logits, int64_t ld_n, int64_t ld_t, const int64_t* targets, int64_t tg_sn,
+                                  const int64_t* lens1, const float* lse, float smoothing, float* loss_rows, const float* mu1,
+                                  const float* lv1, const float* mu2, const float* lv2, int64_t kl_rows, int E, const float* a,
+                                  const float* b, int64_t mse_n, float w_kl, float w_mse, float* partials, float* out, int N, int T,
+                                  int V, void* stream) {
+  ACVAE_TRY(vl_check(logits, targets, lse, mu1, lv1, mu2, lv2, kl_rows, E, a, b, mse_n, N, T, V));
+  if (!loss_rows || !partials || !out) return ACVAE_EINVAL;
+  const int kl_nb = (int)acvae_kl_partials(kl_rows * E), mse_nb = (int)acvae_kl_partials(mse_n);
+  VlArgs p{};
+  p.logits = logits; p.ld_n = ld_n; p.ld_t = ld_t; p.targets = targets; p.tg_sn = tg_sn; p.lens1 = lens1; p.lse = lse;
+  p.smoothing = smoothing; p.loss_rows = loss_rows; p.N = N; p.T = T; p.V = V;
+  p.mu1 = mu1; p.lv1 = lv1; p.mu2 = mu2; p.lv2 = lv2; p.kl_n = kl_rows * E; p.kl_rows = kl_rows; p.kl_part = partials;
+  p.a = a; p.b = b; p.mse_n = mse_n; p.mse_part = partials + kl_nb;
+  p.w_kl = w_kl; p.w_mse = w_mse;
+  VlTable tb;
+  tb.add({VL_CE}); tb.add({VL_KL}); tb.add({VL_MSE});
+  const int blocks = tb.seal([&](const VlJob& j) { return j.kind == VL_CE ? N * T : j.kind == VL_KL ? kl_nb : mse_nb; });
+  hipLaunchKernelGGL(vae_loss_rows_kernel, dim3(blocks), dim3(EW_THREADS), 0, (hipStream_t)stream, tb, p);
+  hipLaunchKernelGGL(vae_loss_final_kernel, dim3(1), dim3(256), 0, (hipStream_t)stream, p, kl_nb, mse_nb, out);
+  ACVAE_LAUNCH_CHECK();
+  return ACVAE_OK;
+}
+extern "C" int acvae_vae_loss_bwd(const float* logits, int64_t ld_n, int64_t ld_t, const int64_t* targets, int64_t tg_sn,
+                                  const int64_t* lens1, const float* lse, float smoothing, const float* mu1, const float* lv1,
+                                  const float* mu2, const float* lv2, int64_t kl_rows, int E, const float* a, const float* b,
+                                  int64_t mse_n, float w_kl, float w_mse, const float* grad_out, float* dlogits, float* dmu1,
+                                  float* dlv1, float* dmu2, float* dlv2, float* da, float* db, int N, int T, int V, void* stream) {
+  ACVAE_TRY(vl_check(logits, targets, lse, mu1, lv1, mu2, lv2, kl_rows, E, a, b, mse_n, N, T, V));
+  if (!grad_out || !dlogits) return ACVAE_EINVAL;
+  VlArgs p{};
+  p.logits = logits; p.ld_n = ld_n; p.ld_t = ld_t; p.targets = targets; p.tg_sn = tg_sn; p.lens1 = lens1; p.lse = lse;
+  p.smoothing = smoothing; p.N = N; p.T = T; p.V = V;
+  p.mu1 = mu1; p.lv1 = lv1; p.mu2 = mu2; p.lv2 = lv2; p.kl_n = kl_rows * E; p.kl_rows = kl_rows;
+  p.a = a; p.b = b; p.mse_n = mse_n; p.w_kl = w_kl; p.w_mse = w_mse;
+  p.grad_out = grad_out; p.dlogits = dlogits; p.dmu1 = dmu1; p.dlv1 = dlv1; p.dmu2 = dmu2; p.dlv2 = dlv2; p.da = da; p.db = db;
+  VlTable tb;
+  tb.add({VL_CE}); tb.add({VL_KL}); tb.add({VL_MSE});
+  const int kl_nb = grid_for(p.kl_n, EW_THREADS), mse_nb = grid_for(mse_n, EW_THREADS);
+  const int blocks = tb.seal([&](const VlJob& j) { return j.kind == VL_CE ? N * T : j.kind == VL_KL ? kl_nb : mse_nb; });
+  hipLaunchKernelGGL(vae_loss_bwd_kernel, dim3(blocks), dim3(EW_THREADS), 0, (hipStream_t)stream, tb, p);
+  ACVAE_LAUNCH_CHECK();
+  return ACVAE_OK;
+}
+
 extern "C" int acvae_row_logsoftmax_argmax(const float* logits, int64_t ld_n, int64_t ld_t, int64_t* argmax,
                                            float* max_logprob, float* lse, int64_t o_sn, int64_t o_st, int N, int T,
                                            int V, void* stream) {
diff --git a/acvae_amd/csrc/rnn.h b/acvae_amd/csrc/rnn.h
--- a/acvae_amd/csrc/rnn.h
+++ b/acvae_amd/csrc/rnn.h
@@ -31,6 +31,7 @@
              int N, int T, int C, hipStream_t st);
 int colsum_rows(const float* x, long ld, int rows, int cols, float* out, int accumulate, hipStream_t st);
 int add_rows(float* dst, long ld_d, const float* src, long ld_s, int rows, int cols, hipStream_t st);
+int add_rows(float* out, long ld_o, const float* a, long ld_a, const float* b, long ld_b, int rows, int cols, hipStream_t st);
 int copy_rows(float* dst, long ld_d, const float* src, long ld_s, int rows, int cols, hipStream_t st);
 struct CopyRowsJob { float* dst; long ld_d; const float* src; long ld_s; int rows, cols; };
 using CopyRowsBatch = JobTable<CopyRowsJob, 8>;
diff --git a/acvae_amd/csrc/rnn.hip b/acvae_amd/csrc/rnn.hip
--- a/acvae_amd/csrc/rnn.hip
+++ b/acvae_amd/csrc/rnn.hip
@@ -246,6 +246,14 @@
     dst[r * ld_d + c] += src[r * ld_s + c];
   }
 }
+__global__ void add_rows_to_kernel(float* __restrict__ out, long ld_o, const float* __restrict__ a, long ld_a,
+                                   const float* __restrict__ b, long ld_b, int rows, int cols) {
+  const long total = (long)rows * cols;
+  for (long i = blockIdx.x * (long)TH + threadIdx.x; i < total; i += (long)gridDim.x * TH) {
+    const int r = (int)(i / cols), c = (int)(i % cols);
+    out[r * ld_o + c] = a[r * ld_a + c] + b[r * ld_b + c];
+  }
+}
 __global__ void copy_rows_kernel(float* __restrict__ dst, long ld_d, const float* __restrict__ src, long ld_s, int rows,
                                  int cols) {
   const long total = (long)rows * cols;
@@ -373,6 +381,10 @@
   LAUNCH(add_rows_kernel, grid1((long)rows * cols), dst, ld_d, src, ld_s, rows, cols);
   ACVAE_LAUNCH_CHECK(); return ACVAE_OK;
 }
+int add_rows(float* out, long ld_o, const float* a, long ld_a, const float* b, long ld_b, int rows, int cols, hipStream_t st) {
+  LAUNCH(add_rows_to_kernel, grid1((long)rows * cols), out, ld_o, a, ld_a, b, ld_b, rows, cols);
+  ACVAE_LAUNCH_CHECK(); return ACVAE_OK;
+}
 int copy_rows(float* dst, long ld_d, const float* src, long ld_s, int rows, int cols, hipStream_t st) {
   LAUNCH(copy_rows_kernel, grid1((long)rows * cols), dst, ld_d, src, ld_s, rows, cols);
   ACVAE_LAUNCH_CHECK(); return ACVAE_OK;
diff --git a/acvae_amd/streams.py b/acvae_amd/streams.py
--- a/acvae_amd/streams.py
+++ b/acvae_amd/streams.py
@@ -5,12 +5,20 @@
 _SCRATCH = {}
 
 
-def scratch_buffer(nbytes, device, tag=None):
-    key = (device.type, device.index, torch.cuda.current_stream(device).cuda_stream, tag)
+def scratch_buffer(nbytes, device, tag=None, first=None):
+    cur = torch.cuda.current_stream(device)
+    key = (device.type, device.index, cur.cuda_stream, tag)
     buf = _SCRATCH.get(key)
     if buf is None or buf.numel() < nbytes:
         _SCRATCH[key] = buf = torch.empty(int(nbytes), dtype=torch.uint8, device=device)
+        if first is not None:
+            first.wait_stream(cur)
     return buf
+
+
+def empty_on(stream, nbytes, device):
+    with torch.cuda.stream(stream):
+        return torch.empty(int(nbytes), dtype=torch.uint8, device=device)
 
 
 def keep(stream, *objs, _seen=None):
diff --git a/acvae_amd/train_util.py b/acvae_amd/train_util.py
--- a/acvae_amd/train_util.py
+++ b/acvae_amd/train_util.py
@@ -168,6 +168,63 @@
     return _CombineLossFn.apply(ce, kl, mse, kl_weight, alpha if mse is not None else 0.0)
 
 
+class _VaeLossFn(torch.autograd.Function):
+
+    @staticmethod
+    def forward(ctx, logits, targets, lens1, smoothing, mu1, lv1, mu2, lv2, a, b, w_kl, w_mse, lse):
+        _lib.require_cuda(logits, mu1, lv1, mu2, lv2, a, b)
+        logits = logits.float()
+        if not logits.is_contiguous():
+            logits = logits.contiguous()
+        N, T, V = logits.shape
+        dev = logits.device
+        targets = targets.to(device=dev, dtype=torch.long)
+        if targets.stride(-1) != 1:
+            targets = targets.contiguous()
+        lens_d = None if lens1 is None else torch.as_tensor(lens1).to(device=dev, dtype=torch.long).contiguous()
+        ts = [t.contiguous().float() for t in (mu1, lv1, mu2, lv2)]
+        E = ts[0].shape[-1]
+        kl_rows = ts[0].numel() // E
+        a, b = a.contiguous().float(), b.contiguous().float()
+        have_lse = lse is not None
+        if not have_lse:
+            lse = torch.empty(N, T, device=dev)
+        rows = torch.empty(N, T, device=dev)
+        part = torch.empty(_lib.call("acvae_kl_partials", kl_rows * E) + _lib.call("acvae_kl_partials", a.numel()), device=dev)
+        out = torch.empty(4, device=dev)
+        st = _lib.current_stream()
+        if not have_lse:
+            _lib.call("acvae_row_logsoftmax_argmax", logits, logits.stride(0), logits.stride(1), None, None, lse, T, 1, N, T, V, st)
+        _lib.call("acvae_vae_loss_fwd", logits, logits.stride(0), logits.stride(1), targets, targets.stride(0), lens_d, lse,
+                  float(smoothing), rows, *ts, kl_rows, E, a, b, a.numel(), float(w_kl), float(w_mse), part, out, N, T, V, st)
+        ctx.ce = (logits, targets, lens_d, lse, float(smoothing))
+        ctx.ts, ctx.kl_rows, ctx.E, ctx.ab, ctx.w = ts, kl_rows, E, (a, b), (float(w_kl), float(w_mse))
+        loss, ce, kl, mse = out[0], out[1], out[2], out[3]
+        ctx.mark_non_differentiable(ce, kl, mse)
+        return loss, ce, kl, mse
+
+    @staticmethod
+    def backward(ctx, g, *_):
+        logits, targets, lens_d, lse, smoothing = ctx.ce
+        N, T, V = logits.shape
+        need = ctx.needs_input_grad
+        dl = torch.empty(N, T, V, device=logits.device)
+        dts = [torch.empty_like(t) if need[4 + i] else None for i, t in enumerate(ctx.ts)]
+        a, b = ctx.ab
+        da = torch.empty_like(a) if need[8] else None
+        db = torch.empty_like(b) if need[9] else None
+        _lib.call("acvae_vae_loss_bwd", logits, logits.stride(0), logits.stride(1), targets, targets.stride(0), lens_d, lse,
+                  smoothing, *ctx.ts, ctx.kl_rows, ctx.E, a, b, a.numel(), *ctx.w, g.contiguous().float().reshape(1), dl, *dts,
+                  da, db, N, T, V, _lib.current_stream())
+        return (dl, None, None, None, *dts, da, db, None, None, None)
+
+
+def vae_loss(logits, targets, lens1, smoothing, q_means, q_logs, p_means, p_logs, q_means_utt, p_means_utt, kl_weight, alpha,
+             lse=None):
+    return _VaeLossFn.apply(logits, targets, lens1, smoothing, q_means, q_logs, p_means, p_logs, q_means_utt, p_means_utt,
+                            kl_weight, alpha, lse)
+
+
 class MSELoss(nn.Module):
 
     def forward(self, a, b):
diff --git a/acvae_amd/trainer.py b/acvae_amd/trainer.py
--- a/acvae_amd/trainer.py
+++ b/acvae_amd/trainer.py
@@ -8,7 +8,7 @@
 
 from . import _lib, streams
 from .optim import FlatOptimizer, check_group, resolve
-from .train_util import LabelSmoothingLoss, MSELoss, Normal_kl_loss, combine_losses
+from .train_util import LabelSmoothingLoss, MSELoss, Normal_kl_loss, combine_losses, vae_loss
 
 
 class FlatGradExchange:
@@ -108,6 +108,7 @@
         self.criterion = LabelSmoothingLoss(vocab_size, self.smoothing)
         self.kl_loss = Normal_kl_loss()
         self.mse_loss = MSELoss()
+        self.batched_loss = True
         self.pg = process_group
         self.data_parallel = data_parallel
         self.world = dist.get_world_size(process_group) if self._dist() else 1
@@ -239,6 +240,11 @@
             lens1 = np.asarray(cap_lens) - 1
         caps_src = staged.get("caps_d")
         targets = (caps if caps_src is None else caps_src)[:, 1:1 + out["logits"].shape[1]].to(torch.long)
+        if self.alpha is not None and self.batched_loss:
+            loss, ce, kl, mse = vae_loss(out["logits"], targets, lens1, self.criterion.smoothing, out["q_means"], out["q_logs"],
+                                         out["p_means"], out["p_logs"], out["q_means_utt"], out["p_means_utt"], kl_weight,
+                                         self.alpha, lse=staged.pop("lse", None))
+            return loss, {"ce": ce, "kl": kl, "mse": mse}, out
         ce = self.criterion.masked(out["logits"], targets, lens1)
         kl = self.kl_loss(out["q_means"], out["q_logs"], out["p_means"], out["p_logs"])
         mse = None
diff --git a/acvae_amd/vae_model.py b/acvae_amd/vae_model.py
--- a/acvae_amd/vae_model.py
+++ b/acvae_amd/vae_model.py
@@ -27,8 +27,14 @@
         scratch_b = _lib.call("acvae_decode_scratch_bytes", *dims)
         if saved_b < 0:
             raise RuntimeError(f"decode: unsupported dims {dims}")
-        saved = torch.empty(saved_b, dtype=torch.uint8, device=dev)
-        scratch = scratch_buffer(scratch_b, dev)
+        pre = sampling.get("pre") if sampling else None
+        if pre is not None and pre["dims"] == dims:
+            saved, scratch = pre["saved"], pre["scratch"]
+            streams.hand_over(saved, pre["done"])
+        else:
+            pre = None
+            saved = torch.empty(saved_b, dtype=torch.uint8, device=dev)
+            scratch = scratch_buffer(scratch_b, dev)
         f = lambda *s: torch.empty(*s, device=dev)
         logits, outputs = f(N, Tc, V), f(N, Tc, H)
         seqs = torch.empty(N, Tc, dtype=torch.long, device=dev)
@@ -57,7 +63,12 @@
                   mem_lens_d, caps_d, caps_d.stride(0) if train else 0, lens1_d, q_z, eps_p, ss_arr, dis_arr, logits,
                   outputs, seqs, slp, attw, pm, pl, pz, putt, hfin, hp, cp, saved, saved_b, scratch, scratch_b, *dims, model.start_idx,
                   model.end_idx, _lib.current_stream(), model._aux_stream(), int(method), float(temp), noise, keep,
-                  float(drop_p), _lib.call_flags() | (_lib.FLAG_ROLLOUT_GRAD if rollout else 0), *extra)
+                  float(drop_p), _lib.call_flags() | (_lib.FLAG_ROLLOUT_GRAD if rollout else 0) |
+                  (_lib.FLAG_PRE_DONE if pre is not None else 0), *extra)
+        model._decode_lse = None
+        if train and logits.is_contiguous():
+            off = _lib.call("acvae_decode_saved_lse_offset", *dims)
+            model._decode_lse = saved[off:off + N * Tc * 4].view(torch.float32).view(N, Tc)
         ctx.set_materialize_grads(False)
         ctx.model, ctx.saved, ctx.dims, ctx.dis_arr = model, saved, dims, dis_arr
         ctx.emb_keep, ctx.emb_p, ctx.rollout = keep, float(drop_p), rollout
@@ -366,6 +377,7 @@
                 if share is not None:
                     encoded = self._share_rows(encoded, *share)
                 qnetout = on_side(self.qnet, prep["caps_d"], cap_lens, eps=eps_q, keep=q_keep)
+                self._decode_pre(encoded["audio_embeds"], qnetout["q_z"], prep, main, side)
             encoded["_prep"] = prep
             encoded.update(qnetout)
             return self.train_forward(encoded, caps, cap_lens, **kwargs)
@@ -374,6 +386,34 @@
             encoded = self.encoder(feats, feat_lens)
             return self.inference_forward(encoded, **kwargs)
         raise Exception("Number of input should be either 4 (feats, feat_lens, caps, cap_lens) or 2 (feats, feat_lens)")
+
+    def _decode_pre(self, mem, q_z, prep, main, side):
+        if side is main or _lib.options.old_order:
+            return
+        if not all(prep["ss_flags"]) or any(prep["dis_flags"]) or prep["caps_d"] is None:
+            return
+        dec = self.decoder
+        N, S, Eenc = mem.shape
+        dims = (N, prep["Tc"], S, dec.embed_size, dec.model.hidden_size, dec.attn.attn_size, dec.vocab_size, Eenc)
+        saved_b = _lib.call("acvae_decode_saved_bytes", *dims)
+        scratch_b = _lib.call("acvae_decode_scratch_bytes", *dims)
+        if saved_b < 0:
+            return
+        dev = mem.device
+        aux = self.streams.get("decode", main)
+        after_posterior = torch.cuda.Event()
+        after_posterior.record(side)
+        aux.wait_event(after_posterior)
+        saved = streams.empty_on(aux, saved_b, dev)
+        scratch = scratch_buffer(scratch_b, dev, tag="decode", first=aux)
+        sampling = prep["sampling"]
+        keep, drop_p = sampling["emb_keep"] if sampling.get("emb_keep") else (None, 0.0)
+        caps_d = prep["caps_d"]
+        _lib.call_keeping(aux, "acvae_decode_fwd_pre", self._text_table(), caps_d, caps_d.stride(0), q_z.detach(), saved,
+                          saved_b, scratch, scratch_b, *dims, aux.cuda_stream, keep, float(drop_p), 0)
+        done = torch.cuda.Event()
+        done.record(aux)
+        sampling["pre"] = {"saved": saved, "scratch": scratch, "done": done, "dims": dims}
 
     def _share_rows(self, encoded, index, index_d, offsets_d, rows_d):
         mem, pooled = encoded["audio_embeds"], encoded["audio_embeds_pooled"].detach().contiguous()
@@ -518,10 +558,14 @@
         caps_d, lens1_d = prep["caps_d"], prep["lens1_d"]
         q_z = encoded["q_z"] if train else None
         self.staged = {"caps_d": caps_d, "lens1_d": lens1_d}
+        self._decode_lse = None
         with contextlib.nullcontext() if record else torch.no_grad():
             outs = _DecodeFn.apply(self, mem, mem_lens_d, caps_d, lens1_d, q_z, eps_p, ss_flags, dis_flags, Tc,
                                    prep.get("sampling"), *self._decode_weights())
         logits, outputs, seqs, slp, attw, pm, pl, pz, putt, hfin, hp, cp = outs[:12]
+        if train and self._decode_lse is not None:
+            self.staged["lse"] = self._decode_lse
+        self._decode_lse = None
         output = {"seqs": seqs, "logits": logits, "outputs": outputs, "sampled_logprobs": slp,
                   "attn_weights": attw.transpose(1, 2), "p_means": pm, "p_logs": pl, "p_z": pz,
                   "state": hfin.unsqueeze(0), "hiddens_state": (hp.unsqueeze(0), cp.unsqueeze(0)), "last_z": pz[:, -1]}
diff --git a/include/acvae_hip.h b/include/acvae_hip.h
--- a/include/acvae_hip.h
+++ b/include/acvae_hip.h
@@ -12,6 +12,8 @@
 #define ACVAE_FLAG_DEFER_PARAM_GRADS 2
 #define ACVAE_FLAG_NO_ATTN_SPLIT 4
 #define ACVAE_FLAG_ROLLOUT_GRAD 16
+#define ACVAE_FLAG_OLD_ORDER 32
+#define ACVAE_FLAG_PRE_DONE 64
 #define ACVAE_FLAG_TEST_STALL 8
 
 int acvae_persist_status_register(int device, void* status_words_host);
@@ -29,6 +31,9 @@
 int acvae_gemm_nt_dual_ws(const float* A1, int64_t lda1, const float* B1, int64_t ldb1, int K1, const float* A2,
                           int64_t lda2, const float* B2, int64_t ldb2, int K2, const float* bias, float* C, int64_t ldc,
                           int M, int N, int accumulate, float* ws, int64_t ws_bytes, int reset_tickets, void* stream);
+int acvae_gemm_nt_cols_ws(const float* A, int64_t lda, const float* B, int64_t ldb, int K, const float* bias, float* C,
+                          int64_t ldc, int M, int N, int plan_N, int accumulate, float* ws, int64_t ws_bytes, int reset_tickets,
+                          void* stream);
 int acvae_gemm_nt_pair_c(const float* A0, int64_t lda0, const float* B0, int64_t ldb0, int K0, const float* bias0, float* C0,
                          int64_t ldc0, int N0, int acc0, const float* A1, int64_t lda1, const float* B1, int64_t ldb1, int K1,
                          const float* bias1, float* C1, int64_t ldc1, int N1, int acc1, int M, void* stream);
@@ -119,6 +124,16 @@
 int acvae_mse_bwd(const float* a, const float* b, const float* grad_out, float* da, float* db, int64_t n, void* stream);
 int acvae_loss_combine_fwd(const float* ce, const float* kl, const float* mse, float w_kl, float w_mse, float* out, void* stream);
 int acvae_loss_combine_bwd(const float* grad_out, float w_kl, float w_mse, float* g_ce, float* g_kl, float* g_mse, void* stream);
+int acvae_vae_loss_fwd(const float* logits, int64_t ld_n, int64_t ld_t, const int64_t* targets, int64_t tg_sn,
+                       const int64_t* lens1, const float* lse, float smoothing, float* loss_rows, const float* mu1,
+                       const float* lv1, const float* mu2, const float* lv2, int64_t kl_rows, int E, const float* a,
+                       const float* b, int64_t mse_n, float w_kl, float w_mse, float* partials, float* out, int N, int T,
+                       int V, void* stream);
+int acvae_vae_loss_bwd(const float* logits, int64_t ld_n, int64_t ld_t, const int64_t* targets, int64_t tg_sn,
+                       const int64_t* lens1, const float* lse, float smoothing, const float* mu1, const float* lv1,
+                       const float* mu2, const float* lv2, int64_t kl_rows, int E, const float* a, const float* b,
+                       int64_t mse_n, float w_kl, float w_mse, const float* grad_out, float* dlogits, float* dmu1,
+                       float* dlv1, float* dmu2, float* dlv2, float* da, float* db, int N, int T, int V, void* stream);
 
 #define ACVAE_ENC_NPARAMS 55
 #define ACVAE_ARCH_CNN10 0
@@ -263,6 +278,9 @@
                      float* p_means_utt, float* h_final, float* hp_final, float* cp_final, void* saved,
                      int64_t saved_bytes, void* scratch, int64_t scratch_bytes, int N, int Tc, int S, int E, int H,
                      int A, int V, int Eenc, int start_idx, int end_idx, void* stream, void* aux_stream, int flags);
+int acvae_decode_fwd_pre(const void* const* params, const int64_t* caps, int64_t ld_caps, const float* q_z, void* saved,
+                         int64_t saved_bytes, void* scratch, int64_t scratch_bytes, int N, int Tc, int S, int E, int H, int A,
+                         int V, int Eenc, void* stream, const uint8_t* emb_keep, float emb_drop_p, int flags);
 int acvae_decode_fwd_sampled(const void* const* params, const float* mem_in, const int64_t* mem_lens,
                              const int64_t* caps, int64_t ld_caps, const int64_t* lens1, const float* q_z,
                              const float* eps_p, const int* ss_flags_host, const int* dis_flags_host, float* logits,
```

Result: no change. 2155, median of 6 (+0.5%).
